# ldyken53/gaussian-splatting-wgpu

Measured on AMD Instinct MI355X. Metric: frames/sec, higher is better.
Workload: dtype f32; 1 GPU; bicycle-like synthetic 6.1M gaussians @1920x1080; gaussians=6100000, width=1920, height=1080, tile_size=16, parallelism=single GPU, visible=2430918, processed=15909895, block_evaluated=6068168, sort_passes=1, depth_ordered_emission=True, tight_binning=True, blend_mode=fused, camera=64-step orbit, moved every frame

## Files before the change

### gaussian-splatting-wgpu_amd/csrc/gs_context.hip

```cpp
#include <cmath>
#include <cstdarg>
#include <memory>
#include <new>

#include "gs_runtime.h"

thread_local char g_err[512] = "";
int32_t fail(int32_t code, const char* fmt, ...) {
    va_list ap;
    va_start(ap, fmt);
    vsnprintf(g_err, sizeof(g_err), fmt, ap);
    va_end(ap);
    return code;
}

static uint32_t tiles_f32(uint32_t extent, uint32_t ts) {
    return (uint32_t)std::ceil((float)extent / (float)ts);
}
static uint32_t bits_for(uint64_t v) {
    uint32_t b = 0;
    while (v) { ++b; v >>= 1; }
    return b ? b : 1;
}

GS_EXPORT const char* gs_last_error(void) { return g_err; }
GS_EXPORT int32_t gs_abi_version(void) { return GS_ABI_VERSION; }

int32_t alloc_kv(gs_ctx* c, uint64_t capacity, uint64_t row_cap) {
    if (capacity >= (1ull << 30)) return fail(GS_ERR_CAPACITY, "capacity %llu exceeds 2^30 intersections", (unsigned long long)capacity);
    if (row_cap >= (1ull << 31)) return fail(GS_ERR_CAPACITY, "%llu row items exceed the 2^31 limit", (unsigned long long)row_cap);
    c->gr.valid = false;
    c->keysA.reset(); c->valsA.reset(); c->keysB.reset(); c->valsB.reset(); c->keysU.reset(); c->valsU.reset();
    c->keysG.reset(); c->chunk_table.reset(); c->arena.reset(); c->rows_sorted.reset(); c->M3.reset(); c->ctl_mem.reset();
    c->keysG_valid = false;
    capacity = std::max<uint64_t>(capacity, 4096);
    row_cap = (std::max<uint64_t>(row_cap, 4096) + 15) & ~(uint64_t)15;
    const size_t kb = (size_t)capacity * 4;
    HIP_TRY(hipMalloc(c->keysA.out(), kb));
    HIP_TRY(hipMalloc(c->valsA.out(), kb));
    HIP_TRY(hipMalloc(c->keysB.out(), kb));
    HIP_TRY(hipMalloc(c->valsB.out(), kb));
    HIP_TRY(hipMalloc(c->chunk_table.out(), (size_t)gs_emit_chunks(std::max(capacity, row_cap)) * 4));
    if (c->tight_ok) {
        HIP_TRY(hipMalloc(c->arena.out(), (size_t)row_cap * 12));
        HIP_TRY(hipMalloc(c->rows_sorted.out(), (size_t)row_cap * 12));
        HIP_TRY(hipMalloc(c->M3.out(), (size_t)gs_rows_chunks(row_cap) * 256 * 4));
    }
    const size_t ctl_sz = (sizeof(GsControl) + 255) & ~(size_t)255;
    const size_t scan_sz = (((size_t)gs_scan_blocks(c->n ? c->n : 1) + 1) * 8 + 255) & ~(size_t)255;
    const size_t sort_sz = (size_t)std::max(c->passes, c->tile_passes) * gs_sort_tiles(capacity) * 256 * 4;
    const size_t rows_sz = c->tight_ok ? (size_t)gs_rows_sort_tiles(row_cap) * 256 * 4 : 0;
    const size_t depth_sz = ((size_t)c->T * 4 + 255) & ~(size_t)255;
    c->ctl_bytes = ctl_sz + depth_sz + rows_sz + scan_sz + sort_sz;
    c->ctl_bytes_tight = ctl_sz + depth_sz + rows_sz;
    HIP_TRY(hipMalloc(c->ctl_mem.out(), c->ctl_bytes));
    char* const base = (char*)c->ctl_mem.get();
    c->ctl = (GsControl*)base;
    c->tile_depth = (uint32_t*)(base + ctl_sz);
    c->rows_status = (uint32_t*)(base + ctl_sz + depth_sz);
    c->scan_status = (unsigned long long*)(base + ctl_sz + depth_sz + rows_sz);
    c->sort_status = (uint32_t*)(base + ctl_sz + depth_sz + rows_sz + scan_sz);
    c->capacity = capacity;
    c->row_cap = row_cap;
    c->frame.capacity = (uint32_t)capacity;
    c->frame.row_cap = (uint32_t)row_cap;
    return GS_OK;
}

GS_EXPORT int32_t gs_create(const gs_config* cfg, gs_ctx** out) {
    if (!cfg || !out) return fail(GS_ERR_INVALID_ARGUMENT, "gs_create: null argument");
    if (cfg->struct_size != sizeof(gs_config)) return fail(GS_ERR_INVALID_ARGUMENT, "gs_create: struct_size %u != %zu", cfg->struct_size, sizeof(gs_config));
    if (cfg->width == 0 || cfg->height == 0) return fail(GS_ERR_INVALID_ARGUMENT, "gs_create: empty canvas");
    if (cfg->tile_size != 8 && cfg->tile_size != 16 && cfg->tile_size != 32)
        return fail(GS_ERR_INVALID_ARGUMENT, "gs_create: tile_size must be 8, 16 or 32 (got %u)", cfg->tile_size);
    int ndev = 0;
    if (hipGetDeviceCount(&ndev) != hipSuccess || ndev == 0) return fail(GS_ERR_NO_DEVICE, "gs_create: no HIP device");
    if (cfg->device < 0 || cfg->device >= ndev) return fail(GS_ERR_INVALID_ARGUMENT, "gs_create: device %d of %d", cfg->device, ndev);
    HIP_TRY(hipSetDevice(cfg->device));

    std::unique_ptr<gs_ctx> c(new (std::nothrow) gs_ctx());
    if (!c) return fail(GS_ERR_OUT_OF_MEMORY, "gs_create: host allocation failed");
    c->cfg = *cfg;
    GsFrame& f = c->frame;
    f.width = cfg->width; f.height = cfg->height; f.tile_size = cfg->tile_size;
    f.ntx = tiles_f32(cfg->width, cfg->tile_size);
    f.nty = tiles_f32(cfg->height, cfg->tile_size);
    if (f.ntx >= 32768 || f.nty >= 65536) return fail(GS_ERR_INVALID_ARGUMENT, "gs_create: canvas too large");
    f.col0 = cfg->col_begin;
    f.col1 = cfg->col_end;
    if (f.col0 == 0 && f.col1 == 0) f.col1 = f.ntx;
    if (f.col1 > f.ntx || f.col0 >= f.col1) return fail(GS_ERR_INVALID_ARGUMENT, "gs_create: bad tile-column slab [%u,%u) of %u", f.col0, f.col1, f.ntx);
    f.full = (f.col0 == 0 && f.col1 == f.ntx) ? 1u : 0u;
    f.px0 = f.col0 * f.tile_size;
    f.slab_w = std::min(f.width, f.col1 * f.tile_size) - f.px0;
    c->T = f.ntx * f.nty;
    const uint64_t max_key = ((uint64_t)f.nty * f.ntx + f.ntx) * 1000ull + 999ull;
    if (max_key > 0xFFFFFFFFull) return fail(GS_ERR_INVALID_ARGUMENT, "gs_create: tile ids overflow the 32-bit key (write_tile_ids.wgsl:29)");
    c->key_bits = bits_for(max_key);
    c->passes = (c->key_bits + 7) / 8;
    const uint32_t tbits = bits_for((uint64_t)f.nty * f.ntx + f.ntx);
    c->tile_passes = (tbits + 7) / 8;
    c->tile_bits = (tbits + c->tile_passes - 1) / c->tile_passes;
    c->tile16 = ((uint64_t)f.nty * f.ntx + f.ntx) < 0xFFFFull;
    if ((uint64_t)(f.ntx + 1) * (f.nty + 1) > GS_COUNT_MASK) return fail(GS_ERR_INVALID_ARGUMENT, "gs_create: canvas has too many tiles");
    c->tight_ok = f.ntx <= 255u && f.nty <= 255u;

    hipDeviceProp_t prop;
    HIP_TRY(hipGetDeviceProperties(&prop, cfg->device));
    c->grid_persist = (uint32_t)prop.multiProcessorCount * 4;
    if (cfg->stream) c->stream = (hipStream_t)cfg->stream;
    else { HIP_TRY(hipStreamCreateWithFlags(c->own_stream.out(), hipStreamNonBlocking)); c->stream = c->own_stream; }

    HIP_TRY(hipMalloc(c->ranges.out(), (size_t)c->T * 4));
    HIP_TRY(hipMemset(c->ranges, 0, (size_t)c->T * 4));
    const size_t px = (size_t)f.slab_w * f.height;
    HIP_TRY(hipMalloc(c->rgba8.out(), px * 4));
    HIP_TRY(hipMemset(c->rgba8, 0, px * 4));
    if (cfg->flags & GS_FLAG_F32_TAP) HIP_TRY(hipMalloc(c->rgbf.out(), px * 12));
    if (cfg->flags & GS_FLAG_AUX_OUTPUTS) {
        HIP_TRY(hipMalloc(c->alpha.out(), px * 4));
        HIP_TRY(hipMalloc(c->depth.out(), px * 4));
        HIP_TRY(hipMemset(c->alpha, 0, px * 4));
        HIP_TRY(hipMemset(c->depth, 0, px * 4));
    }
    HIP_TRY(hipHostMalloc(c->h_ctl.out(), sizeof(GsControl), hipHostMallocDefault));
    memset(c->h_ctl, 0, sizeof(GsControl));
    HIP_TRY(hipMalloc(c->d_pxb.out(), 65 * 4));
    HIP_TRY(hipMalloc(c->tileoff.out(), 256 * 256 * 4));
    HIP_TRY(hipMalloc(c->rowtot.out(), 256 * 4));
    HIP_TRY(hipMalloc(c->sticky.out(), 4 * 4));
    HIP_TRY(hipMemset(c->sticky, 0, 4 * 4));
    HIP_TRY(hipHostMalloc(c->h_rep.out(), sizeof(GsReport), hipHostMallocDefault));
    memset(c->h_rep, 0, sizeof(GsReport));
    if (cfg->flags & GS_FLAG_TIMING) {
        for (auto& row : c->ev)
            for (auto& e : row) HIP_TRY(hipEventCreate(e.out()));
        c->have_events = true;
    }
    c->fif = (c->own_stream && f.full) ? 3u : 1u;
    *out = c.release();
    return GS_OK;
}

gs_ctx::~gs_ctx() { drop_graph(this); }

GS_EXPORT int32_t gs_destroy(gs_ctx* c) {
    if (!c) return GS_OK;
    hipSetDevice(c->cfg.device);
    drop_shadows(c);
    if (c->stream) hipStreamSynchronize(c->stream);
    delete c;
    return GS_OK;
}

static int32_t alloc_per_gaussian(gs_ctx* c, uint64_t n, uint64_t min_capacity = 0, uint64_t min_rows = 0) {
    c->gr.valid = false;
    c->scene_own.reset();
    c->scene_mem = nullptr;
    c->n = (uint32_t)n;
    c->frame.n = (uint32_t)n;
    c->have_frame = false;
    c->counts.reset(); c->offsets.reset(); c->grec.reset(); c->rowptr.reset(); c->gsort_scratch.reset(); c->gdata.reset();
    const size_t np = ((size_t)n + 63) & ~(size_t)63;
    HIP_TRY(hipMalloc(c->counts.out(), std::max<size_t>(np * 4, 256)));
    HIP_TRY(hipMalloc(c->offsets.out(), std::max<size_t>(np * 4, 256)));
    HIP_TRY(hipMalloc(c->grec.out(), std::max<size_t>(np * 16, 256)));
    HIP_TRY(hipMalloc(c->rowptr.out(), std::max<size_t>(np * 4, 256)));
    HIP_TRY(hipMalloc(c->gsort_scratch.out(), gs_gsort_scratch_bytes((uint32_t)n)));
    HIP_TRY(hipMalloc(c->gdata.out(), std::max<size_t>((size_t)n * 64, 256)));
    HIP_TRY(hipMemsetAsync(c->gdata, 0, std::max<size_t>((size_t)n * 64, 256), c->stream));
    uint64_t cap = c->cfg.max_intersections ? c->cfg.max_intersections : std::max<uint64_t>(4 * n, 1u << 22);
    cap = std::max<uint64_t>(cap, min_capacity);
    cap = std::min<uint64_t>(cap, (1ull << 30) - 1);
    const uint64_t rows = std::max<uint64_t>(std::max<uint64_t>(2 * n, 1u << 20), min_rows);
    return alloc_kv(c, cap, rows);
}

int32_t scene_alloc(gs_ctx* c, uint64_t n, uint64_t min_capacity, uint64_t min_rows) {
    int32_t rc = alloc_per_gaussian(c, n, min_capacity, min_rows);
    if (rc != GS_OK) return rc;
    const size_t np = ((size_t)n + 63) & ~(size_t)63;
    const size_t sh_end = np * 4 * 4 + np * 32 + (size_t)n * 192, state_at = (sh_end + 255) & ~(size_t)255;
    const size_t bytes = has_state(c) ? state_at + np : sh_end;
    HIP_TRY(hipMalloc(c->scene_own.out(), std::max<size_t>(bytes, 256)));
    c->scene_mem = c->scene_own;
    c->scene_bytes = bytes;
    char* p = (char*)c->scene_mem;
    GsScene& s = c->scene;
    s.px = (float*)p; p += np * 4; s.py = (float*)p; p += np * 4; s.pz = (float*)p; p += np * 4;
    s.smax = (float*)p; p += np * 4;
    s.geo = (float4*)p; p += np * 32;
    s.sh = (float4*)p;
    s.state = nullptr;
    if (has_state(c)) {
        s.state = (const uint8_t*)c->scene_mem + state_at;
        HIP_TRY(hipMemsetAsync((char*)c->scene_mem + state_at, 0, std::max<size_t>(np, 4), c->stream));
    }
    return GS_OK;
}

static int32_t upload_common(gs_ctx* c, const void* d_aos, uint64_t n) {
    int32_t rc = scene_alloc(c, n);
    if (rc != GS_OK) return rc;
    if (n) gs_launch_repack(d_aos, (uint32_t)n, c->scene, c->stream);
    HIP_TRY(hipGetLastError());
    HIP_TRY(hipStreamSynchronize(c->stream));
    return GS_OK;
}

void drop_shadows(gs_ctx* c) {
    for (gs_ctx* s : c->shadows) gs_destroy(s);
    c->shadows.clear();
    c->last = c;
    c->rr = 0;
    c->cap_hint = 0;
    c->row_hint = 0;
}
GS_EXPORT int32_t gs_share_splats(gs_ctx* c, gs_ctx* owner) {
    if (!c || !owner || c == owner) return fail(GS_ERR_INVALID_ARGUMENT, "gs_share_splats: needs two distinct contexts");
    if (c->cfg.device != owner->cfg.device) return fail(GS_ERR_INVALID_ARGUMENT, "gs_share_splats: contexts are on different devices");
    if (!c->is_shadow) drop_shadows(c);
    if (!owner->scene_mem) return fail(GS_ERR_NO_SCENE, "gs_share_splats: the owner holds no splats");
    if (has_state(c) && !has_state(owner))
        return fail(GS_ERR_INVALID_ARGUMENT, "gs_share_splats: this context has GS_FLAG_SPLAT_STATE, the owner keeps no state plane");
    HIP_TRY(hipSetDevice(c->cfg.device));
    if (c->pending) { int32_t rc = wait_one(c); if (rc != GS_OK) return rc; }
    int32_t rc = alloc_per_gaussian(c, owner->n, c->cfg.max_intersections ? 0 : owner->capacity, owner->row_cap);
    if (rc != GS_OK) return rc;
    c->scene_mem = owner->scene_mem;
    c->scene_bytes = owner->scene_bytes;
    c->scene = owner->scene;
    HIP_TRY(hipStreamSynchronize(c->stream));
    return GS_OK;
}

GS_EXPORT int32_t gs_upload_splats_device(gs_ctx* c, const void* d_aos, uint64_t n) {
    if (!c || (!d_aos && n)) return fail(GS_ERR_INVALID_ARGUMENT, "gs_upload_splats_device: null argument");
    if (n >= (1ull << 31)) return fail(GS_ERR_INVALID_ARGUMENT, "gs_upload_splats: too many gaussians");
    HIP_TRY(hipSetDevice(c->cfg.device));
    drop_shadows(c);
    return upload_common(c, d_aos, n);
}

GS_EXPORT int32_t gs_upload_splats(gs_ctx* c, const void* aos, uint64_t n) {
    if (!c || (!aos && n)) return fail(GS_ERR_INVALID_ARGUMENT, "gs_upload_splats: null argument");
    if (n >= (1ull << 31)) return fail(GS_ERR_INVALID_ARGUMENT, "gs_upload_splats: too many gaussians");
    HIP_TRY(hipSetDevice(c->cfg.device));
    drop_shadows(c);
    DevBuf<> d;
    const size_t bytes = (size_t)n * GS_SPLAT_RECORD_BYTES;
    HIP_TRY(hipMalloc(d.out(), std::max<size_t>(bytes, 256)));
    if (bytes) {
        hipError_t e = hipMemcpy(d, aos, bytes, hipMemcpyHostToDevice);
        if (e != hipSuccess) return fail(GS_ERR_HIP, "upload memcpy: %s", hipGetErrorString(e));
    }
    return upload_common(c, d, n);
}

GS_EXPORT int32_t gs_host_alloc(uint64_t bytes, void** out) {
    if (!out) return fail(GS_ERR_INVALID_ARGUMENT, "gs_host_alloc: null argument");
    *out = nullptr;
    HIP_TRY(hipHostMalloc(out, std::max<size_t>((size_t)bytes, 256), hipHostMallocDefault));
    return GS_OK;
}
GS_EXPORT void gs_host_free(void* p) { if (p) hipHostFree(p); }

GS_EXPORT int32_t gs_slab_width(gs_ctx* c, uint32_t* px_begin, uint32_t* px_width) {
    if (!c) return fail(GS_ERR_INVALID_ARGUMENT, "gs_slab_width: null ctx");
    if (px_begin) *px_begin = c->frame.px0;
    if (px_width) *px_width = c->frame.slab_w;
    return GS_OK;
}

static int32_t set_option_one(gs_ctx* c, int32_t key, int64_t value) {
    c->gr.valid = false;
    switch (key) {
    case GS_OPT_FRAME_GRAPH: c->gr.use = (value != 0); return GS_OK;
    case GS_OPT_BLEND_ABLATION: c->blend_ablation = (uint32_t)value & 0x3FFFFu; return GS_OK;
    case GS_OPT_PERSISTENT_GRID: if (value <= 0) break; c->grid_persist = (uint32_t)value; return GS_OK;
    case GS_OPT_RESET_TIMING: c->timed_from = c->frames; c->max_I_seen = 0; c->truncated_frames = 0; return GS_OK;
    case GS_OPT_EMIT_ORDER: if (value < 0 || value > 2) break; c->emit_order = (int)value; return GS_OK;
    case GS_OPT_UNFUSED: return GS_OK;
    case GS_OPT_DEBUG_VIEW: if (value < 0 || value > 4) break; c->debug_view = (uint32_t)value; return GS_OK;
    case GS_OPT_TILE_CULL: c->tile_cull = (value != 0); return GS_OK;
    case GS_OPT_PROJ_CHUNKS: if (value != 0 && value != 2 && value != 4 && value != 8) break; c->tight_nb = (uint32_t)value; return GS_OK;
    case GS_OPT_SELECT_TINT:
        if (!has_state(c)) return fail(GS_ERR_INVALID_ARGUMENT, "gs_set_option: GS_OPT_SELECT_TINT needs GS_FLAG_SPLAT_STATE");
        if (value < 0 || value > 0xFFFFFFFFll) break;
        c->select_tint = (uint32_t)value;
        return GS_OK;
    default: break;
    }
    return fail(GS_ERR_INVALID_ARGUMENT, "gs_set_option: bad key/value %d/%lld", key, (long long)value);
}
GS_EXPORT int32_t gs_set_option(gs_ctx* c, int32_t key, int64_t value) {
    if (!c) return fail(GS_ERR_INVALID_ARGUMENT, "gs_set_option: null ctx");
    if (key == GS_OPT_FRAMES_IN_FLIGHT) {
        if (value < 1 || value > 4) return fail(GS_ERR_INVALID_ARGUMENT, "gs_set_option: frames in flight must be 1..4");
        if (!c->own_stream || !c->frame.full) value = 1;
        int32_t rc = gs_wait(c);
        if (rc != GS_OK && rc != GS_ERR_TRUNCATED) return rc;
        while (c->shadows.size() + 1 > (size_t)value) {
            if (c->last == c->shadows.back()) { c->last = c; }
            gs_destroy(c->shadows.back());
            c->shadows.pop_back();
        }
        c->fif = (uint32_t)value;
        c->rr = 0;
        return GS_OK;
    }
    int32_t rc = set_option_one(c, key, value);
    for (gs_ctx* s : c->shadows) if (rc == GS_OK) rc = set_option_one(s, key, value);
    return rc;
}
```

### gaussian-splatting-wgpu_amd/csrc/gs_frame.hip

```cpp
#include <dlfcn.h>

#include "gs_runtime.h"
#include "gs_tight.h"

namespace {
struct Roctx {
    int (*push)(const char*) = nullptr;
    int (*pop)() = nullptr;
    Roctx() {
        void* h = dlopen("librocprofiler-sdk-roctx.so.1", RTLD_LAZY | RTLD_LOCAL);
        if (!h) h = dlopen("libroctx64.so.4", RTLD_LAZY | RTLD_LOCAL);
        if (h) {
            push = (int (*)(const char*))dlsym(h, "roctxRangePushA");
            pop = (int (*)())dlsym(h, "roctxRangePop");
            if (!push || !pop) push = nullptr, pop = nullptr;
        }
    }
};
Roctx& roctx() { static Roctx r; return r; }
const char* const kStageRange[] = {"gsplat:process_gaussians", "gsplat:exclusive_scan", "gsplat:write_tile_ids", "gsplat:radix_sort",
                                   "gsplat:compute_ranges", "gsplat:compute_tiles"};
}

static inline void mark(gs_ctx* c, int i) {
    if (!c->have_events) return;
    hipEventRecord(c->ev[c->frames % GS_EV_RING][i], c->stream);
    Roctx& r = roctx();
    if (r.push) {
        if (i > 0) r.pop();
        if (i < GS_STAGE_COUNT) r.push(kStageRange[i]);
    }
}

static void mark_cb(void* p, int i) { mark((gs_ctx*)p, i); }

static int32_t record_frame(gs_ctx* c, const GsUniforms& u, bool debug, void* ext_rgba8, bool tight) {
    const GsFrame& f = c->frame;
    hipStream_t st = c->stream;
    FrameNotes& nt = c->notes;
    gs_launch_zero(c->ctl_mem, tight ? c->ctl_bytes_tight : c->ctl_bytes, st);
    c->h_ctl_valid = false;
    if (debug) HIP_TRY(hipMemsetAsync(c->gdata, 0, std::max<size_t>((size_t)c->n * 64, 256), st));
    mark(c, 0);
    gs_preprocess_prepare(c->pre, c->scene, u, f, c->gdata, c->counts, tight, c->arena, c->rowptr, c->ctl, c->tight_nb, has_state(c),
                          tint_of(c->select_tint));
    gs_launch_preprocess(c->pre, st);
    mark(c, 1);
    const bool by_index = !tight && (debug || c->index_order);
    bool keys16 = false;
    if (tight) {
        gs_launch_gsort(c->counts, c->rowptr, c->n, c->gsort_scratch, c->grec, c->chunk_table, (uint32_t)gs_emit_chunks(std::max(c->capacity, c->row_cap)),
                        &c->ctl->num_visible, &c->ctl->num_slots, c->grid_persist, st);
        mark(c, 2);
        gs_launch_rows(c->arena, c->grec, c->chunk_table, c->rows_sorted, c->ctl, c->rows_status, (uint32_t)c->row_cap, c->M3, c->tileoff, c->rowtot, f, c->valsA,
                       c->ranges, c->grid_persist / 4u, c->sticky, c->h_rep, st, mark_cb, c);
        nt.keysS = nullptr;
        nt.valsS = c->valsA;
        mark(c, 4);
    } else if (by_index) {
        gs_launch_scan(c->counts, c->n, c->offsets, c->scan_status, &c->ctl->scan_ticket[0], c->ctl, st);
        mark(c, 2);
        gs_launch_emit(c->gdata, c->counts, c->offsets, nullptr, nullptr, f, c->keysA, c->valsA, c->ctl, st);
    } else {
        gs_launch_gsort(c->counts, nullptr, c->n, c->gsort_scratch, c->grec, c->chunk_table, (uint32_t)gs_emit_chunks(std::max(c->capacity, c->row_cap)),
                        &c->ctl->num_visible, &c->ctl->num_intersections, c->grid_persist, st);
        mark(c, 2);
        gs_launch_emit_balanced(c->gdata, c->grec, c->chunk_table, f, c->keysA, c->valsA, c->ctl, c->grid_persist * 2,
                                c->tile_bits, c->tile_passes, c->tile16, st);
        keys16 = c->tile16;
    }
    if (debug) {
        if (!c->keysU) {
            HIP_TRY(hipMalloc(c->keysU.out(), (size_t)c->capacity * 4));
            HIP_TRY(hipMalloc(c->valsU.out(), (size_t)c->capacity * 4));
        }
        HIP_TRY(hipMemcpyAsync(c->keysU, c->keysA, (size_t)c->capacity * 4, hipMemcpyDeviceToDevice, st));
        HIP_TRY(hipMemcpyAsync(c->valsU, c->valsA, (size_t)c->capacity * 4, hipMemcpyDeviceToDevice, st));
    }
    if (!tight) {
        mark(c, 3);
        if (by_index)
            gs_launch_sort(c->keysA, c->valsA, c->keysB, c->valsB, c->ctl, c->ctl->sort_ticket, &c->ctl->hist[0][0], &c->ctl->num_intersections,
                           (uint32_t)c->capacity, c->passes, 8, 0, c->sort_status, c->grid_persist, false, nullptr, nullptr, st, &nt.keysS, &nt.valsS);
        else
            gs_launch_sort(c->keysA, c->valsA, c->keysB, c->valsB, c->ctl, c->ctl->sort_ticket, &c->ctl->hist[0][0], &c->ctl->num_intersections,
                           (uint32_t)c->capacity, c->tile_passes, c->tile_bits, keys16 ? 0 : 1, c->sort_status, c->grid_persist, true,
                           nullptr, nullptr, st, &nt.keysS, &nt.valsS, keys16);
        mark(c, 4);
        if (keys16) gs_launch_ranges16((const uint16_t*)nt.keysS, c->ctl, (uint32_t)c->capacity, c->T, c->ranges, c->grid_persist * 2, c->sticky, c->h_rep, st);
        else gs_launch_ranges(nt.keysS, c->ctl, (uint32_t)c->capacity, c->T, c->ranges, c->grid_persist * 2, c->sticky, c->h_rep, st);
    }
    nt.last_passes = tight ? 1u : (by_index ? c->passes : c->tile_passes);
    nt.last_by_index = by_index;
    nt.last_keys16 = keys16;
    nt.last_tight = tight;
    mark(c, 5);
    uint32_t* target = ext_rgba8 ? (uint32_t*)ext_rgba8 : c->rgba8.get();
    if ((c->blend_ablation & 0x10000u) && !c->blend_prof) HIP_TRY(hipMalloc(c->blend_prof.out(), (size_t)(1u << 20) * 16));
    const bool aux = (c->cfg.flags & GS_FLAG_AUX_OUTPUTS) != 0;
    const int walkers = gs_launch_blend(c->gdata, nt.valsS, c->ranges, f, target, c->rgbf, aux, c->alpha, c->depth, c->ctl, c->tile_depth,
                                        (c->cfg.flags & GS_FLAG_EXACT_BLEND) != 0, c->blend_ablation & 0xFFFFu, tight, st,
                                        (c->blend_ablation & 0x10000u) ? c->blend_prof.get() : nullptr, &c->blend_prof_blocks);
    if (walkers == -2) return fail(GS_ERR_INVALID_ARGUMENT, "blend: GS_FLAG_AUX_OUTPUTS without its alpha / depth planes");
    if (walkers < 0) return fail(GS_ERR_INVALID_ARGUMENT, "unsupported tile size %u", f.tile_size);
    nt.blend_walkers = (uint32_t)walkers;
    mark(c, 6);
    if (c->debug_view) gs_launch_debug_view(c->ranges, f, c->debug_view, target, st);
    return GS_OK;
}

void drop_graph(gs_ctx* c) {
    if (c->gr.exec) hipGraphExecDestroy(c->gr.exec);
    if (c->gr.graph) hipGraphDestroy(c->gr.graph);
    c->gr.exec = nullptr; c->gr.graph = nullptr; c->gr.pre_node = nullptr;
    c->gr.valid = false;
}

static int32_t enqueue_frame(gs_ctx* c, const GsUniforms& u, bool debug, void* ext_rgba8) {
    hipStream_t st = c->stream;
    if (c->emit_order == 2) {
        const uint64_t saved = c->passes > c->tile_passes ? c->passes - c->tile_passes : 0;
        c->index_order = !(c->have_frame && saved * (uint64_t)c->h_rep->num_intersections >= 1000000ull);
    } else {
        c->index_order = (c->emit_order == 1);
    }
    const bool tight = !debug && c->tile_cull && c->tight_ok && c->n < (1u << GS_ID_BITS);
    const bool graphable = c->gr.use && !debug && !c->have_events && !(c->blend_ablation & 0x10000u) && c->n;
    if (graphable) {
        const GraphKey key{c->index_order, tight, ext_rgba8, c->alpha, c->depth};
        if (!c->gr.exec || !c->gr.valid || !(c->gr.key == key)) {
            if (c->gr.exec) HIP_TRY(hipStreamSynchronize(st));
            drop_graph(c);
            HIP_TRY(hipStreamBeginCapture(st, hipStreamCaptureModeRelaxed));
            const int32_t rc = record_frame(c, u, debug, ext_rgba8, tight);
            const hipError_t e = hipStreamEndCapture(st, &c->gr.graph);
            if (rc != GS_OK) { drop_graph(c); return rc; }
            if (e != hipSuccess || !c->gr.graph) return fail(GS_ERR_HIP, "frame graph capture: %s", hipGetErrorString(e));
            hipGraph_t g = c->gr.graph;
            HIP_TRY(hipGraphInstantiate(&c->gr.exec, g, nullptr, nullptr, 0));
            size_t nn = 0;
            HIP_TRY(hipGraphGetNodes(g, nullptr, &nn));
            std::vector<hipGraphNode_t> nodes(nn);
            HIP_TRY(hipGraphGetNodes(g, nodes.data(), &nn));
            uint32_t found = 0;
            for (hipGraphNode_t nd : nodes) {
                hipGraphNodeType ty;
                if (hipGraphNodeGetType(nd, &ty) != hipSuccess || ty != hipGraphNodeTypeKernel) continue;
                hipKernelNodeParams kp;
                if (hipGraphKernelNodeGetParams(nd, &kp) == hipSuccess && kp.func == c->pre.func) { c->gr.pre_node = nd; ++found; }
            }
            if (found != 1) {
                c->gr.use = false;
                c->gr.pre_node = nullptr;
            }
            c->gr.key = key;
            c->gr.notes = c->notes;
            c->gr.valid = true;
        } else {
            c->notes = c->gr.notes;
            gs_preprocess_prepare(c->pre, c->scene, u, c->frame, c->gdata, c->counts, tight, c->arena, c->rowptr, c->ctl, c->tight_nb, has_state(c),
                                  tint_of(c->select_tint));
            hipKernelNodeParams kp{};
            kp.func = const_cast<void*>(c->pre.func);
            kp.gridDim = dim3(c->pre.blocks); kp.blockDim = dim3(256); kp.sharedMemBytes = 0;
            kp.kernelParams = c->pre.args; kp.extra = nullptr;
            HIP_TRY(hipGraphExecKernelNodeSetParams(c->gr.exec, c->gr.pre_node, &kp));
        }
        HIP_TRY(hipGraphLaunch(c->gr.exec, st));
        c->gr.frames++;
    } else {
        const int32_t rc = record_frame(c, u, debug, ext_rgba8, tight);
        if (rc != GS_OK) return rc;
    }
    c->keysG_valid = false;
    c->h_ctl_valid = false;
    HIP_TRY(hipGetLastError());
    c->pending = true;
    c->have_frame = true;
    c->last_debug = debug;
    c->last_ext = ext_rgba8;
    c->last_u = u;
    c->frames++;
    return GS_OK;
}

static int32_t render_common(gs_ctx* c, const void* uniforms, bool debug, void* ext) {
    if (!c || !uniforms) return fail(GS_ERR_INVALID_ARGUMENT, "gs_render: null argument");
    if (!c->scene_mem) return fail(GS_ERR_NO_SCENE, "gs_render: no splats uploaded");
    HIP_TRY(hipSetDevice(c->cfg.device));
    GsUniforms u;
    static_assert(sizeof(GsUniforms) == GS_UNIFORM_BYTES, "uniform block must be 160 bytes");
    memcpy(&u, uniforms, sizeof(u));
    return enqueue_frame(c, u, debug, ext);
}

int32_t wait_one(gs_ctx* c) {
    if (!c) return fail(GS_ERR_INVALID_ARGUMENT, "gs_wait: null ctx");
    HIP_TRY(hipSetDevice(c->cfg.device));
    uint32_t dropped = 0;
    for (int attempt = 0; attempt < 8; ++attempt) {
        HIP_TRY(hipStreamSynchronize(c->stream));
        c->pending = false;
        if (!c->have_frame) return GS_OK;
        const uint32_t over_frames = c->h_rep->sticky[0], fault_any = c->h_rep->sticky[1];
        const uint64_t max_I = c->h_rep->sticky[2], max_rows = c->h_rep->sticky[3];
        if (over_frames || fault_any || max_I || max_rows) HIP_TRY(hipMemset(c->sticky, 0, 4 * 4));
        c->h_rep->sticky[0] = c->h_rep->sticky[1] = c->h_rep->sticky[2] = c->h_rep->sticky[3] = 0;
        if (max_I > c->max_I_seen) c->max_I_seen = max_I;
        if (fault_any || c->h_rep->fault) return fail(GS_ERR_DEVICE_FAULT, "a look-back spin exceeded its bound (fault word set)");
        const uint64_t I = c->h_rep->num_intersections;
        uint64_t rows_last = 0;
        if (c->notes.last_tight)
            for (int k = 0; k < 16; ++k) rows_last = std::max<uint64_t>(rows_last, (uint64_t)c->h_rep->row_cursor[k] * 16);
        const bool last_over = I > c->capacity || c->h_rep->overflow;
        if (attempt == 0 && over_frames > (last_over ? 1u : 0u)) dropped = over_frames - (last_over ? 1u : 0u);
        const uint64_t need = std::max<uint64_t>(I, max_I), need_rows = std::max<uint64_t>(rows_last, max_rows);
        if (!last_over && need <= c->capacity && need_rows <= c->row_cap) break;
        if (need >= (1ull << 30)) return fail(GS_ERR_CAPACITY, "%llu intersections exceed the 2^30 limit", (unsigned long long)need);
        uint64_t want = c->capacity, want_rows = c->row_cap;
        if (need > c->capacity) want = std::min<uint64_t>(std::max<uint64_t>(need + need / 4, c->capacity * 2), (1ull << 30) - 1);
        if (need_rows > c->row_cap) want_rows = std::max<uint64_t>(need_rows + need_rows / 4, c->row_cap * 2);
        if (want == c->capacity && want_rows == c->row_cap) {
            if (last_over) return fail(GS_ERR_CAPACITY, "the frame reports an overflow that growing cannot fix (capacity %llu, rows %llu)",
                                       (unsigned long long)c->capacity, (unsigned long long)c->row_cap);
            break;
        }
        int32_t rc = alloc_kv(c, want, want_rows);
        if (rc != GS_OK) return rc;
        if (!last_over) break;
        if (attempt == 7) return fail(GS_ERR_CAPACITY, "capacity did not converge");
        c->frames--;
        rc = enqueue_frame(c, c->last_u, c->last_debug, c->last_ext);
        if (rc != GS_OK) return rc;
    }
    if (dropped) {
        c->truncated_frames += dropped;
        return fail(GS_ERR_TRUNCATED, "%u frame(s) enqueued before the last one overflowed the (key,value) capacity and were rendered from "
                    "truncated lists; the capacity has been grown to %llu -- wait after every frame, or pass gs_config.max_intersections",
                    dropped, (unsigned long long)c->capacity);
    }
    return GS_OK;
}

GS_EXPORT int32_t gs_wait(gs_ctx* c) {
    if (!c) return fail(GS_ERR_INVALID_ARGUMENT, "gs_wait: null ctx");
    int32_t first = wait_one(c);
    char msg[sizeof(g_err)];
    if (first != GS_OK) memcpy(msg, g_err, sizeof(msg));
    for (gs_ctx* s : c->shadows) {
        const int32_t rc = wait_one(s);
        if (rc != GS_OK && first == GS_OK) { first = rc; memcpy(msg, g_err, sizeof(msg)); }
    }
    c->cap_hint = std::max(c->cap_hint, c->capacity);
    c->row_hint = std::max(c->row_hint, c->row_cap);
    for (gs_ctx* s : c->shadows) { c->cap_hint = std::max(c->cap_hint, s->capacity); c->row_hint = std::max(c->row_hint, s->row_cap); }
    if (first != GS_OK) memcpy(g_err, msg, sizeof(msg));
    return first;
}

static int32_t add_shadow(gs_ctx* c) {
    gs_config cfg = c->cfg;
    cfg.stream = nullptr;
    cfg.max_intersections = 0;
    gs_ctx* s = nullptr;
    int32_t rc = gs_create(&cfg, &s);
    if (rc != GS_OK) return rc;
    s->fif = 1;
    s->is_shadow = true;
    rc = gs_share_splats(s, c);
    if (rc != GS_OK) { gs_destroy(s); return rc; }
    s->emit_order = c->emit_order; s->tile_cull = c->tile_cull; s->debug_view = c->debug_view;
    s->blend_ablation = c->blend_ablation; s->grid_persist = c->grid_persist; s->timed_from = 0; s->tight_nb = c->tight_nb;
    s->select_tint = c->select_tint;
    s->gr.use = c->gr.use;
    c->shadows.push_back(s);
    return GS_OK;
}

GS_EXPORT int32_t gs_render(gs_ctx* c, const void* uniforms) {
    if (!c || !uniforms) return fail(GS_ERR_INVALID_ARGUMENT, "gs_render: null argument");
    gs_ctx* t = c;
    if (c->fif > 1 && c->scene_mem) {
        if (c->pending && c->shadows.size() + 1 < c->fif) {
            int32_t rc = add_shadow(c);
            if (rc != GS_OK) return rc;
            c->rr = (uint32_t)c->shadows.size();
        }
        if (!c->shadows.empty()) {
            const uint32_t slot = c->rr++ % (uint32_t)(c->shadows.size() + 1);
            t = slot ? c->shadows[slot - 1] : c;
        }
        if (t->capacity < c->cap_hint || t->row_cap < c->row_hint) {
            HIP_TRY(hipSetDevice(t->cfg.device));
            if (t->pending) { int32_t rc = wait_one(t); if (rc != GS_OK && rc != GS_ERR_TRUNCATED) return rc; }
            int32_t rc = alloc_kv(t, std::max(t->capacity, c->cap_hint), std::max(t->row_cap, c->row_hint));
            if (rc != GS_OK) return rc;
            t->have_frame = false;
        }
    }
    const int32_t rc = render_common(t, uniforms, false, nullptr);
    if (rc == GS_OK) c->last = t;
    return rc;
}
GS_EXPORT int32_t gs_render_debug(gs_ctx* c, const void* uniforms) {
    const int32_t rc = render_common(c, uniforms, true, nullptr);
    if (rc == GS_OK && c) c->last = c;
    return rc;
}
GS_EXPORT int32_t gs_render_to(gs_ctx* c, const void* uniforms, void* d_rgba8) {
    if (!d_rgba8) return fail(GS_ERR_INVALID_ARGUMENT, "gs_render_to: null output");
    const int32_t rc = render_common(c, uniforms, false, d_rgba8);
    if (rc == GS_OK && c) c->last = c;
    return rc;
}

GS_EXPORT int32_t gs_render_host(gs_ctx* c, const void* uniforms, void* host_dst, uint64_t size, uint64_t* ticket) {
    if (!c || !uniforms || !host_dst || !ticket) return fail(GS_ERR_INVALID_ARGUMENT, "gs_render_host: null argument");
    const uint64_t bytes = (uint64_t)c->frame.slab_w * c->frame.height * 4;
    if (size < bytes) return fail(GS_ERR_INVALID_ARGUMENT, "gs_render_host: need %llu bytes, got %llu", (unsigned long long)bytes, (unsigned long long)size);
    int32_t rc = gs_render(c, uniforms);
    if (rc != GS_OK) return rc;
    gs_ctx* t = last_of(c);
    if (!t->ev_done) HIP_TRY(hipEventCreateWithFlags(t->ev_done.out(), hipEventDisableTiming));
    HIP_TRY(hipMemcpyAsync(host_dst, t->rgba8, bytes, hipMemcpyDeviceToHost, t->stream));
    std::lock_guard<std::mutex> lk(c->ticket_mu);
    HIP_TRY(hipEventRecord(t->ev_done, t->stream));
    const uint64_t k = c->next_ticket++;
    c->tickets[k & 63u].ticket = k;
    c->tickets[k & 63u].member = t;
    *ticket = k;
    return GS_OK;
}

GS_EXPORT int32_t gs_wait_ticket(gs_ctx* c, uint64_t ticket) {
    if (!c) return fail(GS_ERR_INVALID_ARGUMENT, "gs_wait_ticket: null ctx");
    gs_ctx* t = nullptr;
    {
        std::lock_guard<std::mutex> lk(c->ticket_mu);
        if (ticket == 0 || ticket >= c->next_ticket) return fail(GS_ERR_INVALID_ARGUMENT, "gs_wait_ticket: unknown ticket %llu", (unsigned long long)ticket);
        if (c->next_ticket - ticket > 64 || c->tickets[ticket & 63u].ticket != ticket) return GS_OK;
        t = c->tickets[ticket & 63u].member;
    }
    HIP_TRY(hipSetDevice(c->cfg.device));
    HIP_TRY(hipEventSynchronize(t->ev_done));
    return GS_OK;
}
```

### gaussian-splatting-wgpu_amd/csrc/gs_kernels.h

```cpp
#pragma once
#include "gs_device.h"

void gs_launch_repack(const void* d_aos, uint32_t n, const GsScene& s, hipStream_t st);
void gs_launch_ply_chunk(const void* d_raw, uint32_t m, uint32_t first, const GsPlyTable& t, const GsScene& s, hipStream_t st);
struct GsPreprocessLaunch {
    const void* func;
    uint32_t blocks;
    GsScene s; GsUniforms u; GsFrame f;
    void* gdata; uint32_t* counts; GsTightOut to; GsTint tint;
    void* args[7];
};
void gs_preprocess_prepare(GsPreprocessLaunch& L, const GsScene& s, const GsUniforms& u, const GsFrame& f, void* gdata, uint32_t* counts,
                           bool tight, uint32_t* arena, uint32_t* rowptr, GsControl* ctl, uint32_t tight_nb = 0, bool state = false,
                           GsTint tint = GsTint{});
void gs_launch_preprocess(GsPreprocessLaunch& L, hipStream_t st);
void gs_launch_zero(void* p, uint64_t bytes, hipStream_t st);
uint32_t gs_scan_blocks(uint32_t n);
void gs_launch_scan(const uint32_t* counts, uint32_t n, uint32_t* offsets, unsigned long long* status, uint32_t* ticket, GsControl* ctl,
                    hipStream_t st);
uint64_t gs_emit_chunks(uint64_t capacity);
void gs_launch_emit_balanced(const void* gdata, const void* grec, const uint32_t* chunk_table, const GsFrame& f, uint32_t* keys, uint32_t* values,
                             GsControl* ctl, uint32_t grid, uint32_t hist_bits, uint32_t hist_passes, bool keys16, hipStream_t st);
void gs_launch_emit(const void* gdata, const uint32_t* counts, const uint32_t* offsets, const uint32_t* perm, const uint32_t* n_dev,
                    const GsFrame& f, uint32_t* keys, uint32_t* values, GsControl* ctl, hipStream_t st);
void gs_launch_ranges16(const uint16_t* tiles, const GsControl* ctl, uint32_t capacity, uint32_t T, uint32_t* ranges, uint32_t grid,
                        uint32_t* sticky, GsReport* rep, hipStream_t st);
void gs_launch_rebuild_keys(const uint16_t* tiles, const uint32_t* vals, const uint32_t* counts, uint32_t count, uint32_t n, uint32_t id_mask,
                            uint32_t* keys, hipStream_t st);
void gs_launch_ranges(const uint32_t* keys, const GsControl* ctl, uint32_t capacity, uint32_t T, uint32_t* ranges, uint32_t grid,
                      uint32_t* sticky, GsReport* rep, hipStream_t st);
uint32_t gs_sort_tiles(uint64_t capacity);
void gs_launch_sort(uint32_t* keysA, uint32_t* valsA, uint32_t* keysB, uint32_t* valsB, GsControl* ctl, uint32_t* tickets, uint32_t* hist,
                    const uint32_t* n_ptr, uint32_t capacity, uint32_t passes, uint32_t bits, uint32_t by_tile, uint32_t* status,
                    uint32_t grid, bool have_hist, const uint32_t* aux_table, uint32_t* aux_out, hipStream_t st, uint32_t** out_keys,
                    uint32_t** out_vals, bool keys16 = false);
int gs_launch_blend(const void* gdata, const uint32_t* values, const uint32_t* ranges, const GsFrame& f, uint32_t* rgba8, float* rgbf,
                    bool aux, float* alpha, float* depth, GsControl* ctl, uint32_t* tile_depth, bool exact, uint32_t ablation, bool masked, hipStream_t st, uint32_t* prof = nullptr,
                    uint32_t* prof_blocks = nullptr);
void gs_launch_debug_view(const uint32_t* ranges, const GsFrame& f, uint32_t view, uint32_t* rgba8, hipStream_t st);
void gs_launch_assemble(const void* slabs, void* image, uint32_t width, uint32_t height, const uint32_t* d_px_bounds, uint32_t n_slabs,
                        uint64_t slab_stride_px, hipStream_t st);
uint32_t gs_gsort_tiles(uint32_t n);
uint64_t gs_gsort_scratch_bytes(uint32_t n);
void gs_launch_gsort(const uint32_t* words, const uint32_t* aux_in, uint32_t n, void* scratch, void* grec, uint32_t* chunk_table, uint32_t chunk_cap,
                     uint32_t* tot_visible, uint32_t* tot_quantity, uint32_t grid, hipStream_t st);
uint32_t gs_rows_sort_tiles(uint64_t row_cap);
uint32_t gs_rows_chunks(uint64_t row_cap);
void gs_launch_rows(const uint32_t* arena, const void* grec, const uint32_t* chunk_table, uint32_t* rows_sorted, GsControl* ctl, uint32_t* sort_status, uint32_t row_cap,
                    uint32_t* M3, uint32_t* tileoff, uint32_t* rowtot, const GsFrame& f, uint32_t* values, uint32_t* ranges, uint32_t cus,
                    uint32_t* sticky, GsReport* rep, hipStream_t st, void (*mark)(void*, int), void* mark_arg);
void gs_launch_rows_rebuild_keys(const uint32_t* ranges, uint32_t T, const uint32_t* vals, const uint32_t* counts, uint32_t count, uint32_t n,
                                 uint32_t* keys, hipStream_t st);
struct GsRegionDev {
    float a[3], b[3];
    float x0, y0, x1, y1;
    float W, H;
    uint32_t wi, hi;
    float proj[16];
    float viewz[4];
    const uint8_t* mask;
};
#define GS_STATE_SLOTS 32
#define GS_STATE_SLOT_STRIDE 32
void gs_launch_state_region(uint32_t kind, uint8_t* state, const GsScene& s, uint32_t n, const GsRegionDev& r, uint32_t op, uint32_t bits,
                            uint32_t where_mask, uint32_t where_value, unsigned long long* matched, hipStream_t st);
void gs_launch_state_ids(uint8_t* state, const uint32_t* ids, uint64_t n, uint32_t op, uint32_t bits, hipStream_t st);
void gs_launch_state_count(const uint8_t* state, uint32_t n, uint32_t mask, uint32_t value, unsigned long long* count, hipStream_t st);
uint32_t gs_select_blocks(uint32_t n);
void gs_launch_select_count(const uint8_t* state, uint32_t n, uint32_t mask, uint32_t value, uint32_t* counts, hipStream_t st);
void gs_launch_select_scatter(const uint8_t* state, uint32_t n, uint32_t mask, uint32_t value, const uint32_t* offsets, uint32_t* ids, uint32_t cap,
                              hipStream_t st);
void gs_launch_unpack(const GsScene& s, uint32_t n, const uint32_t* ids, uint32_t first, uint32_t m, void* d_aos, uint32_t* out_ids, hipStream_t st);
void gs_launch_compact_planes(const GsScene& o, uint32_t n_old, const uint32_t* ids, uint32_t m, const GsScene& d, hipStream_t st);
void gs_launch_pick(const void* gdata, const uint32_t* values, const uint32_t* ranges, const GsFrame& f, uint32_t id_mask, const void* d_queries,
                    uint32_t n, void* d_results, uint32_t max_contrib, void* d_contrib, hipStream_t st);
```

### gaussian-splatting-wgpu_amd/csrc/gs_runtime.h

```cpp
#pragma once
#include <hip/hip_runtime.h>

#include <algorithm>
#include <cstdint>
#include <cstdio>
#include <cstring>
#include <mutex>
#include <vector>

#include "../../include/gsplat/gs_abi.h"
#include "gs_kernels.h"

#define GS_EXPORT extern "C" __attribute__((visibility("default")))

extern thread_local char g_err[512];
int32_t fail(int32_t code, const char* fmt, ...) __attribute__((format(printf, 2, 3)));
#define HIP_TRY(expr)                                                                                       \
    do {                                                                                                    \
        hipError_t e_ = (expr);                                                                             \
        if (e_ != hipSuccess)                                                                               \
            return fail(e_ == hipErrorOutOfMemory ? GS_ERR_OUT_OF_MEMORY : GS_ERR_HIP, "%s: %s", #expr,      \
                        hipGetErrorString(e_));                                                             \
    } while (0)

template <class P, auto Destroy>
struct Owned {
    P p = nullptr;
    Owned() = default;
    explicit Owned(P q) : p(q) {}
    Owned(const Owned&) = delete;
    Owned& operator=(const Owned&) = delete;
    Owned(Owned&& o) noexcept : p(o.p) { o.p = nullptr; }
    Owned& operator=(Owned&& o) noexcept { if (this != &o) { reset(); p = o.p; o.p = nullptr; } return *this; }
    ~Owned() { reset(); }
    void reset() { if (p) { (void)Destroy(p); p = nullptr; } }
    P* out() { reset(); return &p; }
    P get() const { return p; }
    operator P() const { return p; }
    P operator->() const { return p; }
};
template <class T = void> using DevBuf = Owned<T*, hipFree>;
template <class T = void> using PinnedBuf = Owned<T*, hipHostFree>;
using Event = Owned<hipEvent_t, hipEventDestroy>;
using Stream = Owned<hipStream_t, hipStreamDestroy>;
using File = Owned<FILE*, fclose>;

struct FrameNotes {
    uint32_t *keysS = nullptr, *valsS = nullptr;
    uint32_t last_passes = 0;
    uint32_t blend_walkers = 1;
    bool last_by_index = true;
    bool last_keys16 = false;
    bool last_tight = false;
};

struct GraphKey {
    bool index = false, tight = false;
    void* ext = nullptr;
    float *alpha = nullptr, *depth = nullptr;
    bool operator==(const GraphKey& o) const { return index == o.index && tight == o.tight && ext == o.ext && alpha == o.alpha && depth == o.depth; }
};

#define GS_EV_RING 256
struct gs_ctx {
    ~gs_ctx();
    gs_config cfg{};
    Stream own_stream;
    hipStream_t stream = nullptr;
    GsFrame frame{};
    uint32_t T = 0, passes = 0, key_bits = 0;
    uint32_t tile_passes = 0, tile_bits = 0;
    bool tile16 = false;
    bool tight_ok = false;
    uint32_t grid_persist = 0;
    int emit_order = 2;
    bool index_order = true;
    uint32_t debug_view = 0;
    bool tile_cull = true;
    uint32_t tight_nb = 0;
    uint32_t blend_ablation = 0;
    uint32_t select_tint = 0x80FFFF00u;
    DevBuf<uint32_t> blend_prof;
    uint32_t blend_prof_blocks = 0;
    uint32_t fif = 1;
    std::vector<gs_ctx*> shadows;
    bool is_shadow = false;
    gs_ctx* last = nullptr;
    uint32_t rr = 0;
    uint64_t cap_hint = 0, row_hint = 0;
    Event ev_done;
    uint64_t next_ticket = 1;
    struct { uint64_t ticket; gs_ctx* member; } tickets[64] = {};
    std::mutex ticket_mu;
    DevBuf<> scene_own;
    void* scene_mem = nullptr;
    size_t scene_bytes = 0;
    GsScene scene{};
    uint32_t n = 0;
    DevBuf<uint32_t> counts, offsets, rowptr;
    DevBuf<> gdata;
    DevBuf<> grec;
    DevBuf<> gsort_scratch;
    uint64_t capacity = 0;
    DevBuf<uint32_t> keysA, valsA, keysB, valsB;
    DevBuf<uint32_t> keysU, valsU;
    DevBuf<uint32_t> keysG;
    bool keysG_valid = false;
    DevBuf<uint32_t> chunk_table;
    uint64_t row_cap = 0;
    DevBuf<uint32_t> arena, rows_sorted, M3;
    DevBuf<uint32_t> tileoff, rowtot;
    DevBuf<> ctl_mem;
    size_t ctl_bytes = 0;
    size_t ctl_bytes_tight = 0;
    GsControl* ctl = nullptr;
    uint32_t* tile_depth = nullptr;
    uint32_t* rows_status = nullptr;
    unsigned long long* scan_status = nullptr;
    uint32_t* sort_status = nullptr;
    PinnedBuf<GsControl> h_ctl;
    bool h_ctl_valid = false;
    PinnedBuf<GsReport> h_rep;
    DevBuf<uint32_t> sticky;
    uint64_t max_I_seen = 0;
    uint64_t truncated_frames = 0;
    DevBuf<uint32_t> ranges, rgba8;
    DevBuf<float> rgbf;
    DevBuf<float> alpha, depth;
    DevBuf<uint32_t> d_pxb;
    uint32_t pxb_host[65] = {};
    uint32_t pxb_n = 0;
    struct { DevBuf<> q, r, c; uint64_t c_bytes = 0; } pick;
    struct { DevBuf<unsigned long long> counter; DevBuf<uint32_t> ids; DevBuf<uint8_t> mask; uint64_t ids_cap = 0, mask_cap = 0; } st;
    struct { DevBuf<uint32_t> counts, ids; uint64_t counts_cap = 0, ids_cap = 0; } ex;
    Event ev[GS_EV_RING][GS_STAGE_COUNT + 1];
    bool have_events = false;
    uint64_t timed_from = 0;
    struct {
        bool use = false, valid = false;
        hipGraph_t graph = nullptr;
        hipGraphExec_t exec = nullptr;
        hipGraphNode_t pre_node = nullptr;
        GraphKey key;
        FrameNotes notes;
        uint64_t frames = 0;
    } gr;
    GsPreprocessLaunch pre{};
    FrameNotes notes;
    bool have_frame = false, pending = false, last_debug = false;
    void* last_ext = nullptr;
    GsUniforms last_u{};
    uint64_t frames = 0;
};

int32_t alloc_kv(gs_ctx* c, uint64_t capacity, uint64_t row_cap);
int32_t scene_alloc(gs_ctx* c, uint64_t n, uint64_t min_capacity = 0, uint64_t min_rows = 0);
void drop_shadows(gs_ctx* c);
void drop_graph(gs_ctx* c);
int32_t wait_one(gs_ctx* c);
inline gs_ctx* last_of(gs_ctx* c) { return (c && c->last) ? c->last : c; }
inline bool has_state(const gs_ctx* c) { return (c->cfg.flags & GS_FLAG_SPLAT_STATE) != 0; }
inline GsTint tint_of(uint32_t argb) {
    return GsTint{{(float)((argb >> 16) & 255u) / 255.0f, (float)((argb >> 8) & 255u) / 255.0f, (float)(argb & 255u) / 255.0f},
                  (float)(argb >> 24) / 255.0f};
}
```

### gaussian-splatting-wgpu_amd/csrc/gs_tight.h

```cpp
#pragma once
#include "gs_device.h"

#define GS_ID_BITS 28
#define GS_ID_MASK 0x0FFFFFFFu

struct TightG {
    float gx, gy;
    float cx, cy, cz;
    float cxz;
    float lim2;
    float rcx;
    float xmax, ymax;
    float dyR, eR;
    float kc, qa, qb;
    uint32_t mode;
};

__device__ __forceinline__ bool tight_finite(float x) { return __builtin_fabsf(x) < 3.0e38f; }

__device__ __forceinline__ TightG tight_setup(float uvx, float uvy, float cx, float cy, float cz, float op, float Wf, float Hf) {
    TightG g;
    g.gx = uvx * Wf;
    g.gy = uvy * Hf;
    g.cx = cx; g.cy = cy; g.cz = cz;
    g.cxz = cx * cz;
    const float cyy = cy * cy;
    const float D = g.cxz - cyy;
    const float errD = 4.0e-7f * (g.cxz + cyy);
    const float lim = __builtin_amdgcn_logf(op * 255.0f) * 0.693147182464599609375f + 0.01f;
    g.lim2 = 2.0f * lim;
    g.rcx = 1.0f / cx;
    g.xmax = 0.0f; g.ymax = 0.0f; g.dyR = 0.0f; g.eR = 0.0f;
    g.kc = -(cy * g.rcx);
    g.qa = (cyy - g.cxz) + 1.0e-5f * (cyy + g.cxz);
    g.qb = (g.lim2 * cx) * 1.00001f;
    const bool pd = (cx > 0.0f) && (cz > 0.0f) && (D > 0.0f);
    const bool fin = tight_finite(g.gx) && tight_finite(g.gy) && tight_finite(cx) && tight_finite(cy) && tight_finite(cz) && tight_finite(g.rcx);
    if (!fin) { g.mode = 2u; return g; }
    if (lim < 0.0f) { g.mode = 0u; return g; }
    const float Dlo = D - 1.1e-5f * (g.cxz + cyy) - errD;
    if (!pd || !fin || !tight_finite(lim) || !(Dlo > 0.25f * D)) { g.mode = 2u; return g; }
    g.xmax = __builtin_sqrtf(g.lim2 * 1.0001f * cz / Dlo) * 1.0002f + 0.02f;
    g.ymax = __builtin_sqrtf(g.lim2 * 1.0001f * cx / Dlo) * 1.0002f + 0.02f;
    g.dyR = -cy * g.xmax / cz;
    g.eR = __builtin_fabsf(g.dyR) * ((D - Dlo) / Dlo + 4.0e-4f) + 0.02f;
    g.mode = tight_finite(g.xmax) && tight_finite(g.ymax) && tight_finite(g.dyR) ? 1u : 2u;
    return g;
}

__device__ __forceinline__ bool tight_chord(const TightG& g, float dy, float& xlo, float& xhi) {
    const float up = __builtin_fmaf(dy * dy, g.qa, g.qb);
    if (!(up >= 0.0f)) return false;
    const float hw = __builtin_amdgcn_sqrtf(up) * g.rcx;
    const float c = g.kc * dy;
    xlo = c - hw;
    xhi = c + hw;
    return true;
}

__device__ __forceinline__ bool tight_strip(const TightG& g, float a, float b, bool va, float lo_a, float hi_a, bool vb, float lo_b,
                                            float hi_b, float& plo, float& phi) {
    float xlo, xhi;
    if (!va && !vb) {
        if (!(a <= 0.0f && 0.0f <= b)) return false;
        xlo = -g.xmax;
        xhi = g.xmax;
    } else {
        xlo = va ? (vb ? __builtin_fminf(lo_a, lo_b) : lo_a) : lo_b;
        xhi = va ? (vb ? __builtin_fmaxf(hi_a, hi_b) : hi_a) : hi_b;
        if (g.dyR >= a - g.eR && g.dyR <= b + g.eR) xhi = g.xmax;
        if (-g.dyR >= a - g.eR && -g.dyR <= b + g.eR) xlo = -g.xmax;
    }
    const float slack = 0.02f + 1.0e-5f * (__builtin_fabsf(xlo) + __builtin_fabsf(xhi) + __builtin_fabsf(g.gx));
    plo = g.gx - xhi - slack;
    phi = g.gx - xlo + slack;
    return true;
}

__device__ __forceinline__ void tight_cols(float plo, float phi, float w, float inv_w, int cmin, int cmax, int& lo, int& hi) {
    const float flo = __builtin_ceilf((plo - (w - 1.0f)) * inv_w), fhi = __builtin_floorf(phi * inv_w);
    lo = flo <= (float)cmin ? cmin : (flo > (float)cmax ? cmax + 1 : (int)flo);
    hi = fhi >= (float)cmax ? cmax : (fhi < (float)cmin ? cmin - 1 : (int)fhi);
}

struct TightChord { bool v; float lo, hi; };
__device__ __forceinline__ TightChord tight_chord_at(const TightG& g, float dy) {
    TightChord c;
    c.lo = c.hi = 0.0f;
    c.v = tight_chord(g, dy, c.lo, c.hi);
    return c;
}
__device__ __forceinline__ float tight_row_dy(const TightG& g, uint32_t ty, uint32_t ts) { return g.gy - (float)(ty * ts); }

__device__ __forceinline__ void tight_rows(const TightG& g, uint32_t y0, uint32_t y1, uint32_t ts, float inv_ts, uint32_t nty, uint32_t alias,
                                           uint32_t& ra, uint32_t& rb) {
    if (y1 > nty) y1 = nty;
    ra = y0; rb = y1 > y0 ? y1 : y0;
    if (g.mode != 1u) return;
    const float lo = __builtin_floorf((g.gy - g.ymax) * inv_ts) - (alias ? 1.0f : 0.0f), hi = __builtin_floorf((g.gy + g.ymax) * inv_ts) + 1.0f;
    if (lo > (float)ra) ra = lo >= (float)rb ? rb : (uint32_t)lo;
    if (hi < (float)rb) rb = hi <= (float)ra ? ra : (uint32_t)hi;
}

struct TightRow { int tlo, thi; uint32_t alias; };
__device__ __forceinline__ uint32_t tight_row(const TightG& g, uint32_t ty, uint32_t ts, float inv_ts, uint32_t nty, uint32_t xa, uint32_t wmain,
                                              uint32_t alias, const TightChord& cb, const TightChord& ca, TightRow& r) {
    r.tlo = 0; r.thi = -1; r.alias = 0u;
    if (ty >= nty) return 0u;
    if (wmain) {
        if (g.mode == 2u) { r.tlo = (int)xa; r.thi = (int)(xa + wmain) - 1; }
        else {
            float plo, phi;
            if (tight_strip(g, tight_row_dy(g, ty + 1u, ts), tight_row_dy(g, ty, ts), ca.v, ca.lo, ca.hi, cb.v, cb.lo, cb.hi, plo, phi))
                tight_cols(plo, phi, (float)ts, inv_ts, (int)xa, (int)(xa + wmain) - 1, r.tlo, r.thi);
            else { r.tlo = (int)xa; r.thi = (int)xa - 1; }
        }
    }
    if (alias && ty + 1u < nty) {
        if (g.mode == 2u) r.alias = 1u;
        else {
            const TightChord c2 = tight_chord_at(g, tight_row_dy(g, ty + 2u, ts));
            float plo, phi;
            int lo = 1, hi = 0;
            if (tight_strip(g, tight_row_dy(g, ty + 2u, ts), tight_row_dy(g, ty + 1u, ts), c2.v, c2.lo, c2.hi, ca.v, ca.lo, ca.hi, plo, phi))
                tight_cols(plo, phi, (float)ts, inv_ts, 0, 0, lo, hi);
            r.alias = lo <= hi ? 1u : 0u;
        }
    }
    return (uint32_t)(r.thi >= r.tlo ? r.thi - r.tlo + 1 : 0) + r.alias;
}

__device__ __forceinline__ uint32_t tight_count(const TightG& g, uint32_t y0, uint32_t y1, uint32_t ts, float inv_ts, uint32_t nty, uint32_t xa,
                                                uint32_t wmain, uint32_t alias) {
    if (g.mode == 0u) return 0u;
    uint32_t ra, rb, n = 0;
    tight_rows(g, y0, y1, ts, inv_ts, nty, alias, ra, rb);
    if (ra >= rb) return 0u;
    TightRow r;
    TightChord cb = tight_chord_at(g, tight_row_dy(g, ra, ts));
    for (uint32_t ty = ra; ty < rb; ++ty) {
        const TightChord ca = tight_chord_at(g, tight_row_dy(g, ty + 1u, ts));
        n += tight_row(g, ty, ts, inv_ts, nty, xa, wmain, alias, cb, ca, r);
        cb = ca;
    }
    return n;
}

__device__ __forceinline__ void tight_substrips(const TightG& g, uint32_t ty, uint32_t ts, uint32_t sub, float inv_sub, int cmin, int cmax,
                                                const TightChord& cb, const TightChord& ca, int lo[2], int hi[2]) {
    lo[0] = lo[1] = cmax + 1; hi[0] = hi[1] = cmin - 1;
    if (g.mode == 2u) { lo[0] = lo[1] = cmin; hi[0] = hi[1] = cmax; return; }
    const float yb = tight_row_dy(g, ty, ts), ya = tight_row_dy(g, ty + 1u, ts);
    float plo, phi;
    if (sub == ts) {
        if (tight_strip(g, ya, yb, ca.v, ca.lo, ca.hi, cb.v, cb.lo, cb.hi, plo, phi)) tight_cols(plo, phi, (float)sub, inv_sub, cmin, cmax, lo[0], hi[0]);
        return;
    }
    const float ym = g.gy - (float)(ty * ts + sub);
    const TightChord cm = tight_chord_at(g, ym);
    if (tight_strip(g, ym, yb, cm.v, cm.lo, cm.hi, cb.v, cb.lo, cb.hi, plo, phi)) tight_cols(plo, phi, (float)sub, inv_sub, cmin, cmax, lo[0], hi[0]);
    if (tight_strip(g, ya, ym, ca.v, ca.lo, ca.hi, cm.v, cm.lo, cm.hi, plo, phi)) tight_cols(plo, phi, (float)sub, inv_sub, cmin, cmax, lo[1], hi[1]);
}

#define GS_ROW_HOLE 0xFFFFFFFFu
#define GS_ROW_MAX_DIM 255u
__device__ __forceinline__ uint32_t tight_enc8(int v) { return v <= 0 ? 0u : (v >= 255 ? 255u : (uint32_t)v); }
__device__ __forceinline__ uint32_t tight_pack_intervals(const int lo[2], const int hi[2], int cmin, uint32_t ncols) {
    if (ncols > 254u) return 0xFF00FF00u;
    uint32_t w = 0;
#pragma unroll
    for (int s = 0; s < 2; ++s) {
        uint32_t l = 0, h = 0;
        if (lo[s] <= hi[s]) { l = tight_enc8(lo[s] - cmin); h = tight_enc8(hi[s] + 1 - cmin); }
        w |= (l | (h << 8)) << (16 * s);
    }
    return w;
}
__device__ __forceinline__ uint32_t tight_slot_item(const TightG& g, uint32_t slot, uint32_t ra, uint32_t nrows, uint32_t ts, float inv_ts, uint32_t sub,
                                                    float inv_sub, uint32_t ns, uint32_t nty, uint32_t xa, uint32_t wmain, uint32_t alias, uint32_t& w1,
                                                    uint32_t& w2) {
    w1 = 0u; w2 = 0u;
    TightRow r;
    int lo[2], hi[2];
    if (slot < nrows) {
        const uint32_t ty = ra + slot;
        if (ty >= nty || !wmain) return 0u;
        const int cmin = (int)(xa * ns), cmax = (int)((xa + wmain) * ns) - 1;
        const TightChord cb = tight_chord_at(g, tight_row_dy(g, ty, ts)), ca = tight_chord_at(g, tight_row_dy(g, ty + 1u, ts));
        tight_substrips(g, ty, ts, sub, inv_sub, cmin, cmax, cb, ca, lo, hi);
        int slo = cmax + 1, shi = cmin - 1;
#pragma unroll
        for (int h = 0; h < 2; ++h)
            if (lo[h] <= hi[h]) { slo = lo[h] < slo ? lo[h] : slo; shi = hi[h] > shi ? hi[h] : shi; }
        if (slo > shi) return 0u;
        const uint32_t tlo = (uint32_t)slo / ns, thi = (uint32_t)shi / ns, len = thi - tlo + 1u;
        w1 = ty | (tlo << 8) | ((len - 1u) << 16);
        w2 = tight_pack_intervals(lo, hi, (int)(tlo * ns), len * ns);
        return len;
    }
    if (!alias) return 0u;
    const uint32_t ty = ra + (slot - nrows);
    const TightChord cb = tight_chord_at(g, tight_row_dy(g, ty, ts)), ca = tight_chord_at(g, tight_row_dy(g, ty + 1u, ts));
    if (!tight_row(g, ty, ts, inv_ts, nty, xa, 0u, 1u, cb, ca, r)) return 0u;
    const TightChord c2 = tight_chord_at(g, tight_row_dy(g, ty + 2u, ts));
    tight_substrips(g, ty + 1u, ts, sub, inv_sub, 0, (int)ns - 1, ca, c2, lo, hi);
    w1 = (ty + 1u);
    w2 = tight_pack_intervals(lo, hi, 0, ns);
    return 1u;
}
__device__ __forceinline__ uint32_t tight_item_mask(uint32_t w2, uint32_t q, uint32_t ns) {
    const uint32_t l0 = w2 & 0xFFu, h0 = (w2 >> 8) & 0xFFu, l1 = (w2 >> 16) & 0xFFu, h1 = w2 >> 24;
    if (ns == 2u) {
        const uint32_t c0 = 2u * q, c1 = c0 + 1u;
        return (uint32_t)(l0 <= c0 && (c0 < h0 || h0 == 255u)) | ((uint32_t)(l0 <= c1 && (c1 < h0 || h0 == 255u)) << 1) |
               ((uint32_t)(l1 <= c0 && (c0 < h1 || h1 == 255u)) << 2) | ((uint32_t)(l1 <= c1 && (c1 < h1 || h1 == 255u)) << 3);
    }
    return (uint32_t)(l0 <= q && (q < h0 || h0 == 255u));
}
```

### gaussian-splatting-wgpu_amd/csrc/k_blend.hip

```cpp
#include "gs_device.h"
#include "gs_tight.h"
#include <type_traits>

__device__ __forceinline__ float block_qmin(float cx, float cy, float cz, float dxlo, float dxhi, float dylo, float dyhi,
                                            float& mag) {
    const float X = __builtin_fminf(__builtin_fmaxf(0.0f, dxlo), dxhi);
    const float Y = __builtin_fminf(__builtin_fmaxf(0.0f, dylo), dyhi);
    float q = 3.0e38f;
    mag = 0.0f;
    if (X == 0.0f && Y == 0.0f) return 0.0f;
    if (X != 0.0f) {
        const float dy = __builtin_fminf(__builtin_fmaxf(-cy * X * __builtin_amdgcn_rcpf(cz), dylo), dyhi);
        const float a = 0.5f * cx * X * X, b = 0.5f * cz * dy * dy, c = cy * X * dy;
        q = a + b + c;
        mag = __builtin_fabsf(a) + __builtin_fabsf(b) + __builtin_fabsf(c);
    }
    if (Y != 0.0f) {
        const float dx = __builtin_fminf(__builtin_fmaxf(-cy * Y * __builtin_amdgcn_rcpf(cx), dxlo), dxhi);
        const float a = 0.5f * cx * dx * dx, b = 0.5f * cz * Y * Y, c = cy * dx * Y;
        const float q2 = a + b + c;
        if (q2 < q) { q = q2; mag = __builtin_fabsf(a) + __builtin_fabsf(b) + __builtin_fabsf(c); }
    }
    return q;
}

__device__ __forceinline__ bool blend_tmax_cull(float cx, float cy, float cz, float op, float dxlo, float dxhi, float dylo, float dyhi, float Tmax) {
    const float ax0 = (0.5f * cx) * dxlo * dxlo, ax1 = (0.5f * cx) * dxhi * dxhi, by0 = (0.5f * cz) * dylo * dylo, by1 = (0.5f * cz) * dyhi * dyhi;
    const float c00 = cy * dxlo * dylo, c01 = cy * dxlo * dyhi, c10 = cy * dxhi * dylo, c11 = cy * dxhi * dyhi;
    const float qmax = __builtin_fmaxf(__builtin_fmaxf(ax0 + by0 + c00, ax0 + by1 + c01), __builtin_fmaxf(ax1 + by0 + c10, ax1 + by1 + c11));
    const float qmag = __builtin_fmaxf(ax0, ax1) + __builtin_fmaxf(by0, by1) +
                       __builtin_fmaxf(__builtin_fmaxf(__builtin_fabsf(c00), __builtin_fabsf(c01)), __builtin_fmaxf(__builtin_fabsf(c10), __builtin_fabsf(c11)));
    const float alo = 0.99f * __builtin_fminf(0.99f, op * __builtin_amdgcn_exp2f(-1.44269502162933349609375f * (qmax + 1.0e-5f * qmag)));
    return Tmax * (1.0f - alo) < 0.0000999f;
}

struct GsAuxPlanes { float* alpha; float* depth; };
__device__ __forceinline__ GsAuxPlanes gs_aux_planes() { return GsAuxPlanes{nullptr, nullptr}; }
__device__ __forceinline__ GsAuxPlanes gs_aux_planes(GsAuxPlanes p) { return p; }

template <int TS, bool EXACT, bool AUX = false, typename... Aux>
__global__ __launch_bounds__(TS* TS) void gs_blend_kernel(const uint4* __restrict__ gdata, const uint32_t* __restrict__ values,
                                                           const uint32_t* __restrict__ ranges, GsFrame f,
                                                           uint32_t* __restrict__ rgba8, float* __restrict__ rgbf, GsControl* ctl,
                                                           uint32_t dbg, uint32_t id_mask, Aux... aux) {
    static_assert(sizeof...(Aux) == (AUX ? 1u : 0u), "AUX kernels take one GsAuxPlanes, the others none");
    constexpr int NT = TS * TS;
    constexpr int ROUNDS = NT / 64;
    constexpr int WPR = TS / 8;
    __shared__ float4 sP0[2][NT];
    __shared__ float4 sP1[2][NT];
    __shared__ float4 sP2[2][NT];

    const uint32_t tid = threadIdx.x, lane = tid & 63, w = tid >> 6;
    const uint32_t tx = f.col0 + blockIdx.x, ty = blockIdx.y;
    const uint32_t tile = tx + ty * f.ntx;
    const uint32_t start = tile > 0 ? ranges[tile - 1] : 0u;
    uint32_t end = ranges[tile];
    if (end > f.capacity) end = f.capacity;

    const uint32_t bx0 = tx * TS + (w % WPR) * 8, by0 = ty * TS + (w / WPR) * 8;
    const uint32_t gx = bx0 + (lane & 7), gy = by0 + (lane >> 3);
    const float pxf = (float)gx, pyf = (float)gy;
    const float bx0f = (float)bx0, by0f = (float)by0;
    float T = 1.0f, cr = 0.0f, cg = 0.0f, cb = 0.0f;
    float cd = 0.0f;
    const bool outside = !(gx < f.width && gy < f.height);
    bool done = outside;
    const float c255 = (float)(1.0 / 255.0);
    const float Wf = (float)f.width, Hf = (float)f.height;
    uint32_t staged = 0, evaluated = 0;

    const uint32_t piece = lane & 3u, qrec = lane >> 2;
    uint4 rq[4];
    uint32_t gnext = 0;
    auto fetch_ids = [&](uint32_t b) { gnext = (b + tid < end) ? values[b + tid] : 0u; };
    auto fetch = [&](uint32_t b, uint32_t gval) {
#pragma unroll
        for (int i = 0; i < 4; ++i) {
            const uint32_t rec = qrec + 16u * i;
            uint32_t g = __shfl(gval, rec, 64) & id_mask;
#ifdef GS_PROFILING
            if (dbg & 2u) g &= 1023u;
#endif
            if (b + w * 64u + rec < end && piece < 3u) rq[i] = gdata[(uint64_t)g * 4 + piece];
        }
    };
    auto stage = [&](uint32_t b, int buf) {
#pragma unroll
        for (int i = 0; i < 4; ++i) {
            const uint32_t e = w * 64u + qrec + 16u * i;
            if (b + e < end) {
                const float x = __uint_as_float(rq[i].x), y = __uint_as_float(rq[i].y), z = __uint_as_float(rq[i].z),
                            ww = __uint_as_float(rq[i].w);
                if (piece == 0u) {
                    sP0[buf][e].x = x * Wf;
                    sP0[buf][e].y = y * Hf;
                } else if (piece == 1u) {
                    const float L = 1.44269502162933349609375f;
                    sP1[buf][e] = EXACT ? make_float4(x, y, z, ww) : make_float4((-0.5f * L) * x, (-L) * y, (-0.5f * L) * z, ww);
                } else if (piece == 2u) {
                    sP2[buf][e] = make_float4(x, y, z, ww);
                    sP0[buf][e].z = __builtin_amdgcn_logf(ww * 255.0f) * 0.693147182464599609375f + 0.01f;
                }
            }
        }
    };

    uint32_t gcur = 0;
    if (start < end) {
        fetch_ids(start);
        gcur = gnext;
        fetch(start, gcur);
        fetch_ids(start + NT);
        stage(start, 0);
    }
    __syncthreads();
    int buf = 0;
    for (uint32_t b = start; b < end; b += NT, buf ^= 1) {
        const uint32_t nb = b + NT;
        if (nb < end) {
            gcur = gnext;
            fetch(nb, gcur);
            fetch_ids(nb + NT);
        }
        const uint32_t cnt = (end - b < (uint32_t)NT) ? end - b : (uint32_t)NT;
        staged += cnt;
        const unsigned long long lv = __ballot(!done);
        if (lv != 0ull) {
            uint32_t lcm = (uint32_t)lv | (uint32_t)(lv >> 32);
            lcm |= lcm >> 16; lcm |= lcm >> 8; lcm &= 0xFFu;
            const float lc0 = (float)__builtin_ctz(lcm | 0x100u), lc1 = (float)(31 - __builtin_clz(lcm | 1u));
            const float lr0 = (float)(__builtin_ctzll(lv) >> 3), lr1 = (float)((63 - __builtin_clzll(lv)) >> 3);
            const float Tmax = __uint_as_float((uint32_t)__builtin_amdgcn_readlane((int)wave_incl_max(done ? 0u : __float_as_uint(T)), 63));
#pragma unroll 1
            for (int r = 0; r < ROUNDS; ++r) {
                const uint32_t e0 = (uint32_t)r * 64u;
                if (e0 >= cnt) break;
                bool rel = false;
                if (e0 + lane < cnt) {
                    const float4 p0 = sP0[buf][e0 + lane];
                    float4 p1 = sP1[buf][e0 + lane];
                    if (!EXACT) {
                        const float iL = 0.693147182464599609375f;
                        p1.x *= -2.0f * iL;
                        p1.y *= -iL;
                        p1.z *= -2.0f * iL;
                    }
                    const float dxh = p0.x - bx0f, dyh = p0.y - by0f;
                    const float dxlo = dxh - lc1, dxhi = dxh - lc0, dylo = dyh - lr1, dyhi = dyh - lr0;
                    const bool pd = (p1.x > 0.0f) && (p1.z > 0.0f) && (p1.x * p1.z - p1.y * p1.y > 0.0f);
                    float mag;
                    const float q = block_qmin(p1.x, p1.y, p1.z, dxlo, dxhi, dylo, dyhi, mag);
                    const bool nocull = (dbg & 4u) != 0u;
                    rel = nocull || !pd || !(q > p0.z + 1.0e-5f * mag);
                    if (rel && pd && !nocull && blend_tmax_cull(p1.x, p1.y, p1.z, sP2[buf][e0 + lane].w, dxlo, dxhi, dylo, dyhi, Tmax)) rel = false;
#ifdef GS_PROFILING
                    if (dbg & 1u) rel = false;
#endif
                }
                unsigned long long m = __ballot(rel);
                evaluated += (uint32_t)__popcll(m);
                while (m) {
                    const uint32_t e = e0 + (uint32_t)__builtin_ctzll(m);
                    m &= m - 1ull;
                    const float4 p0 = sP0[buf][e];
                    const float4 p1 = sP1[buf][e];
                    const float4 p2v = sP2[buf][e];
                    const float dx = p0.x - pxf, dy = p0.y - pyf;
                    if (EXACT) {
                        const float t1 = p1.x * dx * dx, t2 = p1.z * dy * dy, t3 = p1.y * dx * dy;
                        const float power = -0.5f * (t1 + t2) - t3;
                        const float alpha = wg_min(0.99f, p2v.w * gs_exp(power));
                        const float test = T * (1.0f - alpha);
                        const float cond = (power <= 0.0f && alpha >= c255 && test >= 0.0001f) ? 1.0f : 0.0f;
                        cr += cond * p2v.x * alpha * T;
                        cg += cond * p2v.y * alpha * T;
                        cb += cond * p2v.z * alpha * T;
                        if constexpr (AUX) cd += cond * p1.w * alpha * T;
                        T = cond * test + (1.0f - cond) * T;
                    } else {
                        const float u = __builtin_fmaf(p1.x, dx, p1.y * dy);
                        const float v = (p1.z * dy) * dy;
                        const float pw = __builtin_fmaf(dx, u, v);
                        const float alpha = __builtin_fminf(0.99f, p2v.w * __builtin_amdgcn_exp2f(pw));
                        const float test = __builtin_fmaf(-T, alpha, T);
                        const bool keep = (pw <= 0.0f) && (alpha >= c255) && (test >= 0.0001f);
                        const float ak = keep ? alpha : 0.0f;
                        const float wgt = ak * T;
                        cr = __builtin_fmaf(p2v.x, wgt, cr);
                        cg = __builtin_fmaf(p2v.y, wgt, cg);
                        cb = __builtin_fmaf(p2v.z, wgt, cb);
                        if constexpr (AUX) cd = __builtin_fmaf(p1.w, wgt, cd);
                        T = keep ? test : T;
                    }
                }
            }
            if (EXACT) done = outside || (T * (1.0f - c255) < 0.0001f);
            else done = outside || (__builtin_fmaf(-T, c255, T) < 0.0001f);
        }
        if (nb < end) stage(nb, buf ^ 1);
        if (__syncthreads_and(done ? 1 : 0)) break;
    }
    if (tid == 0 && staged) atomicAdd(&ctl->num_processed[(blockIdx.x + blockIdx.y * gridDim.x) & 63u], (unsigned long long)staged);
    if (lane == 0 && evaluated) atomicAdd(&ctl->num_evaluated[(blockIdx.x + blockIdx.y * gridDim.x + w) & 63u], (unsigned long long)evaluated);

    if (!outside) {
        const float c[3] = {cr, cg, cb};
        uint32_t q = 0xFF000000u;
#pragma unroll
        for (int ch = 0; ch < 3; ++ch) {
            float v = c[ch];
            v = (v != v) ? 0.0f : wg_min(wg_max(v, 0.0f), 1.0f);
            q |= (uint32_t)__builtin_floorf(v * 255.0f + 0.5f) << (8 * ch);
        }
        const uint64_t o = (uint64_t)gy * f.slab_w + (gx - f.px0);
        rgba8[o] = q;
        if (rgbf) {
            rgbf[o * 3 + 0] = cr;
            rgbf[o * 3 + 1] = cg;
            rgbf[o * 3 + 2] = cb;
        }
        if constexpr (AUX) {
            const GsAuxPlanes ap = gs_aux_planes(aux...);
            ap.alpha[o] = 1.0f - T;
            ap.depth[o] = cd;
        }
    }
}

#ifdef GS_PROFILING
__device__ unsigned long long gs_blend_foot[256][16];
extern "C" __attribute__((visibility("default"))) int gs_prof_blend_footprint(unsigned long long* out4, int reset) {
    static unsigned long long h[256][16];
    if (out4) {
        if (hipMemcpyFromSymbol(h, HIP_SYMBOL(gs_blend_foot), sizeof(h)) != hipSuccess) return -1;
        for (int k = 0; k < 11; ++k) { out4[k] = 0; for (int c = 0; c < 256; ++c) out4[k] += h[c][k]; }
    }
    if (reset) { for (auto& r : h) for (auto& v : r) v = 0; if (hipMemcpyToSymbol(HIP_SYMBOL(gs_blend_foot), h, sizeof(h)) != hipSuccess) return -1; }
    return 0;
}
#endif
constexpr bool gs_lds_disjoint(int a, int na, int b, int nb) { return a + na <= b || b + nb <= a; }
typedef uint32_t gs_u32x2 __attribute__((ext_vector_type(2)));
typedef uint32_t gs_u32x3 __attribute__((ext_vector_type(3)));
typedef uint32_t gs_u32x4 __attribute__((ext_vector_type(4)));
template <bool EXACT, int TS = 16, bool MASKED = false, bool AUX = false, typename... Aux>
__global__ __launch_bounds__(64) void gs_blend_quad_kernel(const uint4* __restrict__ gdata, const uint32_t* __restrict__ values,
                                                            const uint32_t* __restrict__ ranges, GsFrame f,
                                                            uint32_t* __restrict__ rgba8, float* __restrict__ rgbf, GsControl* ctl,
                                                            uint32_t* __restrict__ tile_depth, uint32_t dbg, uint32_t* __restrict__ prof,
                                                            Aux... aux) {
    static_assert(sizeof...(Aux) == (AUX ? 1u : 0u), "AUX kernels take one GsAuxPlanes, the others none");
    constexpr uint32_t BPR = TS / 8, NB = BPR * BPR;
#ifdef GS_PROFILING
    const uint32_t t_start = prof ? (uint32_t)__builtin_amdgcn_s_memrealtime() : 0u;
#endif
#ifndef GS_L_OFF_T
#define GS_L_OFF_T 0
#define GS_L_OFF_Q 4160
#define GS_L_OFF_P 5184
#define GS_L_OFF_L 6208
#define GS_L_TOTAL 6464
#endif
#define GS_L_OFF_Z GS_L_TOTAL
#define GS_L_TOTAL_AUX (GS_L_TOTAL + 256)
    static_assert(gs_lds_disjoint(GS_L_OFF_T, 8 * 65 * 8, GS_L_OFF_Q, 256 * 4) && gs_lds_disjoint(GS_L_OFF_T, 8 * 65 * 8, GS_L_OFF_P, 64 * 16) &&
                  gs_lds_disjoint(GS_L_OFF_T, 8 * 65 * 8, GS_L_OFF_L, 64 * 4) && gs_lds_disjoint(GS_L_OFF_T, 8 * 65 * 8, GS_L_OFF_Z, 64 * 4) &&
                  gs_lds_disjoint(GS_L_OFF_Q, 256 * 4, GS_L_OFF_P, 64 * 16) && gs_lds_disjoint(GS_L_OFF_Q, 256 * 4, GS_L_OFF_L, 64 * 4) &&
                  gs_lds_disjoint(GS_L_OFF_Q, 256 * 4, GS_L_OFF_Z, 64 * 4) && gs_lds_disjoint(GS_L_OFF_P, 64 * 16, GS_L_OFF_L, 64 * 4) &&
                  gs_lds_disjoint(GS_L_OFF_P, 64 * 16, GS_L_OFF_Z, 64 * 4) && gs_lds_disjoint(GS_L_OFF_L, 64 * 4, GS_L_OFF_Z, 64 * 4),
                  "fused LDS regions overlap");
    static_assert(GS_L_OFF_T + 8 * 65 * 8 <= GS_L_TOTAL && GS_L_OFF_Q + 256 * 4 <= GS_L_TOTAL && GS_L_OFF_P + 64 * 16 <= GS_L_TOTAL &&
                  GS_L_OFF_L + 64 * 4 <= GS_L_TOTAL && GS_L_OFF_Z + 64 * 4 <= GS_L_TOTAL_AUX && GS_L_OFF_P % 16 == 0 && GS_L_OFF_T % 8 == 0,
                  "a fused LDS region ends outside its array");
    __shared__ __attribute__((aligned(16))) unsigned char lds_x[EXACT ? 4096 : 16];
    __shared__ __attribute__((aligned(16))) unsigned char lds_f[EXACT ? 16 : (AUX ? GS_L_TOTAL_AUX : GS_L_TOTAL)];
    float4* const sP0 = reinterpret_cast<float4*>(EXACT ? lds_x : lds_f + GS_L_OFF_P);
    float4* const sP1 = reinterpret_cast<float4*>(lds_x + (EXACT ? 1024 : 0));
    float4* const sP2 = reinterpret_cast<float4*>(lds_x + (EXACT ? 2048 : 0));
    uint32_t* const sQ = reinterpret_cast<uint32_t*>(EXACT ? lds_x + 3072 : lds_f + GS_L_OFF_Q);
    float* const sL = reinterpret_cast<float*>(lds_f + (EXACT ? 0 : GS_L_OFF_L));
    float2* const sT = reinterpret_cast<float2*>(lds_f + (EXACT ? 0 : GS_L_OFF_T));
    float* const sZ = reinterpret_cast<float*>(lds_f + ((EXACT || !AUX) ? 0 : GS_L_OFF_Z));
    const uint32_t lane = threadIdx.x;
    const uint32_t slab_tx = f.col1 - f.col0;
    const uint32_t b = blockIdx.x;
    const uint32_t x = b & 7u, j = b >> 3, q = j % NB, t = j / NB;
    const uint32_t SW = (dbg >> 8) & 0xffu;
    const uint32_t ns = (slab_tx + SW - 1) / SW;
    if (x >= ns) return;
    const uint32_t n_x = (ns - 1 - x) / 8 + 1;
    const uint32_t lastw = slab_tx - (ns - 1) * SW;
    const uint32_t Wx = n_x * SW - ((((ns - 1) & 7u) == x) ? SW - lastw : 0u);
    if (t >= Wx * f.nty) return;
    const uint32_t ty = t / Wx, cc = t % Wx;
    const uint32_t tx = f.col0 + (x + 8u * (cc / SW)) * SW + cc % SW;
    const uint32_t lin = ty * slab_tx + (tx - f.col0);
    const uint32_t tile = tx + ty * f.ntx;
    const uint32_t start = tile > 0 ? ranges[tile - 1] : 0u;
    uint32_t end = ranges[tile];
    if (end > f.capacity) end = f.capacity;
    const float c255 = (float)(1.0 / 255.0);
    const float Wf = (float)f.width, Hf = (float)f.height;
    const uint32_t bx0 = tx * TS + (q % BPR) * 8u, by0 = ty * TS + (q / BPR) * 8u;
    const uint32_t gx = bx0 + (lane & 7), gy = by0 + (lane >> 3);
    const float pxf = (float)gx, pyf = (float)gy, bx0f = (float)bx0, by0f = (float)by0;
    const bool outside = !(gx < f.width && gy < f.height);
    bool done = outside;
    float T = 1.0f, cr = 0.0f, cg = 0.0f, cb = 0.0f;
    float cd = 0.0f;
    uint32_t staged = 0, evaluated = 0;
#ifdef GS_PROFILING
    uint32_t fp_lanes = 0, fp_quads = 0, fp_none = 0, fp_live = 0, fp_kept = 0, fp_dead = 0, fp_q1 = 0, fp_tailn = 0, fp_tailbits = 0, fp_nokeep = 0;
#endif

    using R1 = std::conditional_t<AUX, gs_u32x4, gs_u32x3>;
    gs_u32x2 r0 = {0u, 0u};
    R1 r1 = {0u, 0u, 0u};
    gs_u32x4 r2 = {0u, 0u, 0u, 0u};
    const uint32_t mybit = GS_ID_BITS + (TS == 32 ? ((q / BPR) / 2u) * 2u + ((q % BPR) / 2u) : q);
    uint32_t qhead = 0, qn = 0;
    uint32_t pos = start;
    uint32_t g0 = 0, g1 = 0, g2 = 0;
    const __amdgpu_buffer_rsrc_t list_rsrc = __builtin_amdgcn_make_buffer_rsrc((void*)(values + start), 0, (int)((end - start) * 4u), 0x00020000);
    const uint32_t lane4 = lane * 4u;
    auto load_ids = [&]() {
        const uint32_t so = (pos - start) * 4u;
        g0 = __builtin_amdgcn_raw_buffer_load_b32(list_rsrc, lane4, so, 0);
        g1 = __builtin_amdgcn_raw_buffer_load_b32(list_rsrc, lane4 + 256u, so, 0);
        g2 = __builtin_amdgcn_raw_buffer_load_b32(list_rsrc, lane4 + 512u, so, 0);
    };
    const uint32_t mybitmask = 1u << mybit;
    auto push = [&](uint32_t v, uint32_t first) {
        bool want;
        if (MASKED) want = (v & mybitmask) != 0u;
        else want = first + lane < end;
        const unsigned long long m = __ballot(want);
        if (want) sQ[__builtin_amdgcn_mbcnt_hi((uint32_t)(m >> 32), __builtin_amdgcn_mbcnt_lo((uint32_t)m, qhead + qn)) & 255u] = v;
        qn += (uint32_t)__popcll(m);
    };
    auto fill = [&]() {
        while (qn < 64u && pos < end) {
            push(g0, pos); push(g1, pos + 64u); push(g2, pos + 128u);
            const uint32_t adv = end - pos < 192u ? end - pos : 192u;
            staged += adv;
            pos += adv;
            if (pos < end) load_ids();
        }
        __builtin_amdgcn_fence(__ATOMIC_RELEASE, "wavefront");
        __builtin_amdgcn_fence(__ATOMIC_ACQUIRE, "wavefront");
    };
    auto take = [&](uint32_t& v) -> uint32_t {
        const uint32_t cnt = qn < 64u ? qn : 64u;
        v = sQ[(qhead + lane) & 255u];
        qhead = (qhead + cnt) & 255u;
        qn -= cnt;
        return cnt;
    };
    auto fetch = [&](uint32_t v, uint32_t cnt) {
        uint32_t g = MASKED ? (v & GS_ID_MASK) : v;
#ifdef GS_PROFILING
        if (dbg & 2u) g &= 1023u;
#endif
        g = lane < cnt ? g : 0u;
        const uint32_t* rec = reinterpret_cast<const uint32_t*>(gdata + (uint64_t)g * 4);
        r0 = *reinterpret_cast<const gs_u32x2*>(rec);
        r1 = *reinterpret_cast<const R1*>(rec + 4);
        r2 = *reinterpret_cast<const gs_u32x4*>(rec + 8);
    };
    uint32_t cnt = 0, vnext = 0;
    if (start < end) {
        load_ids();
        fill();
        cnt = take(vnext);
        fetch(vnext, cnt);
    }
    while (cnt) {
        bool rel = false, npd = false;
        asm volatile("" : "+v"(r0), "+v"(r1), "+v"(r2));
        const float gxp = __uint_as_float(r0.x) * Wf, gyp = __uint_as_float(r0.y) * Hf;
        const float cx = __uint_as_float(r1.x), cy = __uint_as_float(r1.y), cz = __uint_as_float(r1.z);
        const float op = __uint_as_float(r2.w);
        float z = 0.0f;
        if constexpr (AUX) z = __uint_as_float(r1.w);
        const unsigned long long lv = __ballot(!done);
        uint32_t lcm = (uint32_t)lv | (uint32_t)(lv >> 32);
        lcm |= lcm >> 16; lcm |= lcm >> 8; lcm &= 0xFFu;
        const float lc0 = (float)__builtin_ctz(lcm | 0x100u), lc1 = (float)(31 - __builtin_clz(lcm | 1u));
        const float lr0 = (float)(__builtin_ctzll(lv | (1ull << 63)) >> 3), lr1 = (float)((63 - __builtin_clzll(lv | 1ull)) >> 3);
        const float Tmax = __uint_as_float((uint32_t)__builtin_amdgcn_readlane((int)wave_incl_max(done ? 0u : __float_as_uint(T)), 63));
        if (lane < cnt) {
            const float lim = __builtin_amdgcn_logf(op * 255.0f) * 0.693147182464599609375f + 0.01f;
            const bool pd = (cx > 0.0f) && (cz > 0.0f) && (cx * cz - cy * cy > 0.0f);
            {
                const float dxh = gxp - bx0f, dyh = gyp - by0f;
                float mag;
                const float qm = block_qmin(cx, cy, cz, dxh - lc1, dxh - lc0, dyh - lr1, dyh - lr0, mag);
                const bool nocull = (dbg & 4u) != 0u;
                rel = lv != 0ull && (nocull || !pd || !(qm > lim + 1.0e-5f * mag));
#ifndef GS_NO_TMAX
                if (rel && pd && !nocull) {
                    const float x0 = dxh - lc1, x1 = dxh - lc0, y0 = dyh - lr1, y1 = dyh - lr0;
                    const float ax0 = (0.5f * cx) * x0 * x0, ax1 = (0.5f * cx) * x1 * x1, by0 = (0.5f * cz) * y0 * y0, by1 = (0.5f * cz) * y1 * y1;
                    const float c00 = cy * x0 * y0, c01 = cy * x0 * y1, c10 = cy * x1 * y0, c11 = cy * x1 * y1;
                    const float qmax = __builtin_fmaxf(__builtin_fmaxf(ax0 + by0 + c00, ax0 + by1 + c01), __builtin_fmaxf(ax1 + by0 + c10, ax1 + by1 + c11));
                    const float qmag = __builtin_fmaxf(ax0, ax1) + __builtin_fmaxf(by0, by1) +
                                       __builtin_fmaxf(__builtin_fmaxf(__builtin_fabsf(c00), __builtin_fabsf(c01)), __builtin_fmaxf(__builtin_fabsf(c10), __builtin_fabsf(c11)));
                    const float alo = 0.99f * __builtin_fminf(0.99f, op * __builtin_amdgcn_exp2f(-1.44269502162933349609375f * (qmax + 1.0e-5f * qmag)));
                    if (Tmax * (1.0f - alo) < 0.0000999f) rel = false;
                }
#endif
#ifdef GS_BLEND_PIXTEST
                if (rel && pd && !nocull && (uint32_t)__popcll(lv) <= GS_BLEND_PIXTEST) {
                    bool any = false;
                    for (unsigned long long mm = lv; mm; mm &= mm - 1ull) {
                        const int pl = __builtin_ctzll(mm);
                        const float Tp = __uint_as_float((uint32_t)__builtin_amdgcn_readlane((int)__float_as_uint(T), pl));
                        const float dx = dxh - (float)(pl & 7), dy = dyh - (float)(pl >> 3);
                        const float a = (0.5f * cx) * dx * dx, b = (0.5f * cz) * dy * dy, c = cy * dx * dy;
                        const float q = a + b + c, mg = 1.0e-5f * (a + b + __builtin_fabsf(c));
                        const float ahi = 1.01f * (op * __builtin_amdgcn_exp2f(-1.44269502162933349609375f * (q - mg)));
                        const float alo = 0.99f * __builtin_fminf(0.99f, op * __builtin_amdgcn_exp2f(-1.44269502162933349609375f * (q + mg)));
                        any = any || !(ahi < c255 || Tp * (1.0f - alo) < 0.0000999f);
                    }
                    rel = any;
                }
#endif
            }
#ifdef GS_PROFILING
            if (dbg & 1u) rel = false;
#endif
            npd = rel && !pd;
        }
#ifdef GS_PROFILING
        if ((dbg & 32u) && MASKED && __popcll(lv) <= 16) {
            const unsigned long long rm = __ballot(rel);
            const uint32_t bits = __popc((vnext >> GS_ID_BITS) & 15u);
            fp_tailn += (uint32_t)__popcll(rm);
            fp_tailbits += (uint32_t)__popcll(__ballot(rel && bits >= 1u)) + (uint32_t)__popcll(__ballot(rel && bits >= 2u)) + (uint32_t)__popcll(__ballot(rel && bits >= 3u)) + (uint32_t)__popcll(__ballot(rel && bits >= 4u));
        }
#endif
        const unsigned long long m = __ballot(rel);
        if (rel) {
            const uint32_t slot = __builtin_amdgcn_mbcnt_hi((uint32_t)(m >> 32), __builtin_amdgcn_mbcnt_lo((uint32_t)m, 0u));
            const float L = 1.44269502162933349609375f;
            if (EXACT) {
                sP0[slot] = make_float4(gxp, gyp, 0.0f, 0.0f);
                sP1[slot] = make_float4(cx, cy, cz, z);
                sP2[slot] = make_float4(__uint_as_float(r2.x), __uint_as_float(r2.y), __uint_as_float(r2.z), op);
            } else {
                const float hx = (-0.5f * L) * cx, hy = (-L) * cy, hz = (-0.5f * L) * cz;
                const float lop = __builtin_amdgcn_logf(op) + 0.014499569695115089f;
                const float d = gxp - bx0f;
                const float b0 = (-2.0f * hx) * d, a1 = hy * d, a0 = __builtin_fmaf(hx * d, d, lop);
                sP0[slot] = make_float4(hx, 0.99f * __uint_as_float(r2.x), 0.99f * __uint_as_float(r2.y), 0.99f * __uint_as_float(r2.z));
                sL[slot] = lop;
                if constexpr (AUX) sZ[slot] = 0.99f * z;
#pragma unroll
                for (int r = 0; r < 8; ++r) {
                    const float dy = gyp - (by0f + (float)r);
                    sT[r * 65 + slot] = make_float2(__builtin_fmaf(-hy, dy, b0), __builtin_fmaf(dy, __builtin_fmaf(dy, hz, a1), a0));
                }
            }
        }
        fill();
        const uint32_t cnt_next = take(vnext);
        if (cnt_next) fetch(vnext, cnt_next);
        __builtin_amdgcn_fence(__ATOMIC_RELEASE, "wavefront");
        __builtin_amdgcn_fence(__ATOMIC_ACQUIRE, "wavefront");
        const uint32_t nrel = (uint32_t)__popcll(m);
        evaluated += nrel;
        const uint32_t trow = (lane >> 3) * 65u;
        const float xlf = (float)(lane & 7u);
        auto walk = [&](auto checked_tag) {
            constexpr bool CHECKED = decltype(checked_tag)::value;
            auto one = [&](uint32_t e, const float4 p0, const float2 tt, const float zz) {
                if (EXACT) {
                    const float dx = p0.x - pxf;
                    const float4 p1 = sP1[e];
                    const float dy = p0.y - pyf;
                    const float4 p2v = sP2[e];
                    const float t1 = p1.x * dx * dx, t2 = p1.z * dy * dy, t3 = p1.y * dx * dy;
                    const float power = -0.5f * (t1 + t2) - t3;
                    const float alpha = wg_min(0.99f, p2v.w * gs_exp(power));
                    const float test = T * (1.0f - alpha);
                    const float cond = (power <= 0.0f && alpha >= c255 && test >= 0.0001f) ? 1.0f : 0.0f;
                    cr += cond * p2v.x * alpha * T;
                    cg += cond * p2v.y * alpha * T;
                    cb += cond * p2v.z * alpha * T;
                    if constexpr (AUX) cd += cond * p1.w * alpha * T;
                    T = cond * test + (1.0f - cond) * T;
                } else {
                    const float pw = __builtin_fmaf(xlf, __builtin_fmaf(xlf, p0.x, tt.x), tt.y);
                    float ea;
                    asm("v_exp_f32_e64 %0, %1 clamp" : "=v"(ea) : "v"(pw));
                    const float k1 = (float)(1.0 / 255.0 / 0.99);
#ifdef GS_PROFILING
                    if (dbg & 32u) {
                        const unsigned long long km = __ballot(ea >= k1);
                        const unsigned long long q0 = 0x000000000F0F0F0Full;
                        fp_lanes += (uint32_t)__popcll(km);
                        fp_quads += (uint32_t)((km & q0) != 0) + (uint32_t)((km & (q0 << 4)) != 0) + (uint32_t)((km & (q0 << 32)) != 0) + (uint32_t)((km & (q0 << 36)) != 0);
                        fp_none += (uint32_t)(km == 0);
                        const unsigned long long lv = __ballot(__builtin_fmaf(-T, c255, T) >= 0.0001f);
                        const unsigned long long kp = __ballot(ea >= k1 && __builtin_fmaf(T * ea, -0.99f, T) >= 0.0001f);
                        fp_live += (uint32_t)__popcll(lv);
                        fp_kept += (uint32_t)__popcll(kp);
                        fp_dead += (uint32_t)((km & lv) == 0);
                        fp_q1 += (uint32_t)(__popcll(lv) <= 16);
                        fp_nokeep += (uint32_t)(kp == 0ull);
                    }
#endif
                    if (CHECKED) {
                        const float wgt = T * ea;
                        const float test = __builtin_fmaf(wgt, -0.99f, T);
                        bool keep = (ea >= k1) && (test >= 0.0001f);
                        keep = keep && (pw <= sL[e]);
                        const float wk = keep ? wgt : 0.0f;
                        cr = __builtin_fmaf(p0.y, wk, cr);
                        cg = __builtin_fmaf(p0.z, wk, cg);
                        cb = __builtin_fmaf(p0.w, wk, cb);
                        if constexpr (AUX) cd = __builtin_fmaf(zz, wk, cd);
                        T = keep ? test : T;
                    } else {
                        float wgt, test;
                        unsigned long long save;
                        if constexpr (AUX)
                            asm(
                                "v_mul_f32_e32 %[wgt], %[T], %[ea]\n\t"
                                "v_fma_f32 %[test], %[wgt], %[m99], %[T]\n\t"
                                "s_mov_b64 %[save], exec\n\t"
                                "v_cmpx_le_f32_e32 vcc, %[k1], %[ea]\n\t"
                                "v_cmpx_le_f32_e32 vcc, %[thr], %[test]\n\t"
                                "v_mov_b32_e32 %[T], %[test]\n\t"
                                "v_fmac_f32_e32 %[cr], %[c0], %[wgt]\n\t"
                                "v_fmac_f32_e32 %[cg], %[c1], %[wgt]\n\t"
                                "v_fmac_f32_e32 %[cb], %[c2], %[wgt]\n\t"
                                "v_fmac_f32_e32 %[cd], %[z], %[wgt]\n\t"
                                "s_mov_b64 exec, %[save]"
                                : [save] "=&s"(save), [wgt] "=&v"(wgt), [test] "=&v"(test), [T] "+v"(T), [cr] "+v"(cr), [cg] "+v"(cg), [cb] "+v"(cb),
                                  [cd] "+v"(cd)
                                : [k1] "s"(k1), [thr] "s"(0.0001f), [m99] "s"(-0.99f), [ea] "v"(ea), [c0] "v"(p0.y), [c1] "v"(p0.z), [c2] "v"(p0.w),
                                  [z] "v"(zz)
                                : "vcc");
                        else
                        asm(
                            "v_mul_f32_e32 %[wgt], %[T], %[ea]\n\t"
                            "v_fma_f32 %[test], %[wgt], %[m99], %[T]\n\t"
                            "s_mov_b64 %[save], exec\n\t"
                            "v_cmpx_le_f32_e32 vcc, %[k1], %[ea]\n\t"
                            "v_cmpx_le_f32_e32 vcc, %[thr], %[test]\n\t"
                            "v_mov_b32_e32 %[T], %[test]\n\t"
                            "v_fmac_f32_e32 %[cr], %[c0], %[wgt]\n\t"
                            "v_fmac_f32_e32 %[cg], %[c1], %[wgt]\n\t"
                            "v_fmac_f32_e32 %[cb], %[c2], %[wgt]\n\t"
                            "s_mov_b64 exec, %[save]"
                            : [save] "=&s"(save), [wgt] "=&v"(wgt), [test] "=&v"(test), [T] "+v"(T), [cr] "+v"(cr), [cg] "+v"(cg), [cb] "+v"(cb)
                            : [k1] "s"(k1), [thr] "s"(0.0001f), [m99] "s"(-0.99f), [ea] "v"(ea), [c0] "v"(p0.y), [c1] "v"(p0.z), [c2] "v"(p0.w)
                            : "vcc");
                    }
                }
            };
            auto group = [&](uint32_t e, auto n_tag) {
                constexpr int G = decltype(n_tag)::value;
                float4 p[G];
                float2 t[G];
                float zz[G];
#pragma unroll
                for (int k = 0; k < G; ++k) {
                    p[k] = sP0[e + k];
                    t[k] = EXACT ? make_float2(0.0f, 0.0f) : sT[trow + e + k];
                    zz[k] = 0.0f;
                    if constexpr (AUX && !EXACT) zz[k] = sZ[e + k];
                }
                __builtin_amdgcn_sched_barrier(0);
#pragma unroll
                for (int k = 0; k < G; ++k) one(e + k, p[k], t[k], zz[k]);
                __builtin_amdgcn_sched_barrier(0);
            };
            uint32_t e = 0;
            if (!EXACT)
                for (; e + 8u <= nrel; e += 8u) group(e, std::integral_constant<int, 8>{});
            for (; e + 4u <= nrel; e += 4u) group(e, std::integral_constant<int, 4>{});
            for (; e < nrel; ++e) group(e, std::integral_constant<int, 1>{});
        };
        if (EXACT || __ballot(npd) != 0ull) walk(std::true_type{});
        else walk(std::false_type{});
        if (EXACT) done = outside || (T * (1.0f - c255) < 0.0001f);
        else done = outside || (__builtin_fmaf(-T, c255, T) < 0.0001f);
        __builtin_amdgcn_fence(__ATOMIC_RELEASE, "wavefront");
        __builtin_amdgcn_fence(__ATOMIC_ACQUIRE, "wavefront");
        if (__ballot(!done) == 0ull) break;
        cnt = cnt_next;
    }
    if (lane == 0 && staged) atomicMax(&tile_depth[lin], staged);
    if (lane == 0 && evaluated) atomicAdd(&ctl->num_evaluated[(b + 1u) & 63u], (unsigned long long)evaluated);
#ifdef GS_PROFILING
    if ((dbg & 32u) && lane == 0) {
        unsigned long long* fp = gs_blend_foot[b & 255u];
        atomicAdd(&fp[0], (unsigned long long)evaluated); atomicAdd(&fp[1], (unsigned long long)fp_lanes);
        atomicAdd(&fp[2], (unsigned long long)fp_quads); atomicAdd(&fp[3], (unsigned long long)fp_none);
        atomicAdd(&fp[4], (unsigned long long)fp_live); atomicAdd(&fp[5], (unsigned long long)fp_kept);
        atomicAdd(&fp[6], (unsigned long long)fp_dead); atomicAdd(&fp[7], (unsigned long long)fp_q1);
        atomicAdd(&fp[8], (unsigned long long)fp_tailn); atomicAdd(&fp[9], (unsigned long long)fp_tailbits); atomicAdd(&fp[10], (unsigned long long)fp_nokeep);
    }
    if (prof && lane == 0) {
        prof[b * 4u + 0u] = t_start;
        prof[b * 4u + 1u] = (uint32_t)__builtin_amdgcn_s_memrealtime();
        prof[b * 4u + 2u] = evaluated;
        prof[b * 4u + 3u] = staged;
    }
#endif
    if (!outside) {
        const float c[3] = {cr, cg, cb};
        uint32_t px = 0xFF000000u;
#pragma unroll
        for (int ch = 0; ch < 3; ++ch) {
            float v = c[ch];
            v = (v != v) ? 0.0f : wg_min(wg_max(v, 0.0f), 1.0f);
            px |= (uint32_t)__builtin_floorf(v * 255.0f + 0.5f) << (8 * ch);
        }
        const uint64_t o = (uint64_t)gy * f.slab_w + (gx - f.px0);
        rgba8[o] = px;
        if (rgbf) {
            rgbf[o * 3 + 0] = cr;
            rgbf[o * 3 + 1] = cg;
            rgbf[o * 3 + 2] = cb;
        }
        if constexpr (AUX) {
            const GsAuxPlanes ap = gs_aux_planes(aux...);
            ap.alpha[o] = 1.0f - T;
            ap.depth[o] = cd;
        }
    }
}

__global__ __launch_bounds__(256) void gs_assemble_kernel(const uint32_t* __restrict__ slabs, uint32_t* __restrict__ image,
                                                           uint32_t width, uint32_t height, const uint32_t* __restrict__ px_bounds,
                                                           uint32_t n_slabs, uint64_t slab_stride_px) {
    const uint64_t t = (uint64_t)blockIdx.x * 256 + threadIdx.x;
    if (t >= (uint64_t)width * height) return;
    const uint32_t y = (uint32_t)(t / width), x = (uint32_t)(t % width);
    uint32_t g = 0;
    while (g + 1 < n_slabs && x >= px_bounds[g + 1]) ++g;
    const uint32_t x0 = px_bounds[g], w = px_bounds[g + 1] - x0;
    const uint64_t slab_off = slab_stride_px ? (uint64_t)g * slab_stride_px : (uint64_t)x0 * height;
    image[t] = slabs[slab_off + (uint64_t)y * w + (x - x0)];
}

__global__ __launch_bounds__(256) void gs_debug_view_kernel(const uint32_t* __restrict__ ranges, GsFrame f, uint32_t view,
                                                             uint32_t* __restrict__ rgba8) {
    const uint64_t t = (uint64_t)blockIdx.x * 256 + threadIdx.x;
    if (t >= (uint64_t)f.slab_w * f.height) return;
    const uint32_t y = (uint32_t)(t / f.slab_w), x = f.px0 + (uint32_t)(t % f.slab_w);
    const uint32_t tile = x / f.tile_size + (y / f.tile_size) * f.ntx;
    const uint32_t start = tile > 0 ? ranges[tile - 1] : 0u, end = ranges[tile];
    const float len = (float)(end - start);
    float c[3];
    if (view == 1u) {
        if (x % f.tile_size != f.tile_size - 1u && y % f.tile_size != f.tile_size - 1u) return;
        c[0] = 1.0f; c[1] = 0.0f; c[2] = 0.0f;
    } else if (view == 2u) {
        c[0] = c[1] = c[2] = len / 1000.0f;
    } else if (view == 3u) {
        c[0] = (float)x / (float)f.width; c[1] = (float)y / (float)f.height; c[2] = 0.0f;
    } else {
        c[0] = c[1] = len / 100.0f; c[2] = 0.0f;
    }
    uint32_t px = 0xFF000000u;
#pragma unroll
    for (int ch = 0; ch < 3; ++ch) {
        const float v = wg_min(wg_max(c[ch], 0.0f), 1.0f);
        px |= (uint32_t)__builtin_floorf(v * 255.0f + 0.5f) << (8 * ch);
    }
    rgba8[t] = px;
}
void gs_launch_debug_view(const uint32_t* ranges, const GsFrame& f, uint32_t view, uint32_t* rgba8, hipStream_t st) {
    const uint64_t total = (uint64_t)f.slab_w * f.height;
    if (!total || !view) return;
    hipLaunchKernelGGL(gs_debug_view_kernel, dim3((uint32_t)((total + 255) / 256)), dim3(256), 0, st, ranges, f, view, rgba8);
}

template <int TS>
static void launch_blend_t(bool exact, bool aux, GsAuxPlanes ap, dim3 grid, hipStream_t st, const uint4* gdata, const uint32_t* values,
                           const uint32_t* ranges, const GsFrame& f, uint32_t* rgba8, float* rgbf, GsControl* ctl, uint32_t dbg, uint32_t id_mask) {
#define GS_WG(E) hipLaunchKernelGGL((gs_blend_kernel<TS, E>), grid, dim3(TS * TS), 0, st, gdata, values, ranges, f, rgba8, rgbf, ctl, dbg, id_mask)
#define GS_WG_AUX(E) hipLaunchKernelGGL((gs_blend_kernel<TS, E, true, GsAuxPlanes>), grid, dim3(TS * TS), 0, st, gdata, values, ranges, f, rgba8, \
                                        rgbf, ctl, dbg, id_mask, ap)
    if (aux) { if (exact) GS_WG_AUX(true); else GS_WG_AUX(false); }
    else { if (exact) GS_WG(true); else GS_WG(false); }
#undef GS_WG
#undef GS_WG_AUX
}
template <int TS>
static void launch_quad_t(bool exact, bool masked, bool aux, GsAuxPlanes ap, uint32_t nblk, uint32_t pad, hipStream_t st, const uint4* g,
                          const uint32_t* values, const uint32_t* ranges, const GsFrame& f, uint32_t* rgba8, float* rgbf, GsControl* ctl,
                          uint32_t* tile_depth, uint32_t dbg, uint32_t* prof) {
#define GS_QUAD(E, M) hipLaunchKernelGGL((gs_blend_quad_kernel<E, TS, M>), dim3(nblk), dim3(64), pad, st, g, values, ranges, f, rgba8, rgbf, ctl, tile_depth, dbg, prof)
#define GS_QUAD_AUX(E, M) hipLaunchKernelGGL((gs_blend_quad_kernel<E, TS, M, true, GsAuxPlanes>), dim3(nblk), dim3(64), pad, st, g, values, ranges, f, \
                                             rgba8, rgbf, ctl, tile_depth, dbg, prof, ap)
    if (aux) {
        if (exact) { if (masked) GS_QUAD_AUX(true, true); else GS_QUAD_AUX(true, false); }
        else { if (masked) GS_QUAD_AUX(false, true); else GS_QUAD_AUX(false, false); }
    } else {
        if (exact) { if (masked) GS_QUAD(true, true); else GS_QUAD(true, false); }
        else { if (masked) GS_QUAD(false, true); else GS_QUAD(false, false); }
    }
#undef GS_QUAD
#undef GS_QUAD_AUX
}
int gs_launch_blend(const void* gdata, const uint32_t* values, const uint32_t* ranges, const GsFrame& f, uint32_t* rgba8, float* rgbf,
                    bool aux, float* alpha, float* depth, GsControl* ctl, uint32_t* tile_depth, bool exact, uint32_t ablation, bool masked,
                    hipStream_t st, uint32_t* prof, uint32_t* prof_blocks) {
    if (aux && (!alpha || !depth)) return -2;
    const GsAuxPlanes ap{alpha, depth};
    uint32_t dbg = ablation;
    const uint32_t id_mask = masked ? GS_ID_MASK : 0xFFFFFFFFu;
    const dim3 grid(f.col1 - f.col0, f.nty);
    if (grid.x == 0 || grid.y == 0) return 1;
    const uint4* g = (const uint4*)gdata;
    switch (f.tile_size) {
    case 8: launch_blend_t<8>(exact, aux, ap, grid, st, g, values, ranges, f, rgba8, rgbf, ctl, dbg, id_mask); return 1;
    case 16:
    case 32: {
        const bool t32 = f.tile_size == 32;
        if (!(dbg & 8u)) {
            const uint32_t slab_tx = grid.x;
            auto widest = [&](uint32_t sw) {
                const uint32_t ns = (slab_tx + sw - 1) / sw, lastw = slab_tx - (ns - 1) * sw;
                uint32_t wmax = 0;
                for (uint32_t x = 0; x < 8 && x < ns; ++x) {
                    const uint32_t n_x = (ns - 1 - x) / 8 + 1, wx = n_x * sw - ((((ns - 1) & 7u) == x) ? sw - lastw : 0u);
                    wmax = wx > wmax ? wx : wmax;
                }
                return wmax;
            };
            uint32_t SW = (dbg >> 8) & 0xffu;
            if (!SW) {
                SW = 1;
                for (uint32_t sw = 3; sw > 1; --sw)
                    if (widest(sw) * 80u <= slab_tx * 11u) { SW = sw; break; }
            }
            dbg = (dbg & 0xffu) | (SW << 8);
            const uint32_t wmax = widest(SW);
            const uint32_t nblk = (t32 ? 128u : 32u) * wmax * grid.y;
#ifdef GS_PROFILING
            const uint32_t pad = (dbg & 64u) ? 20480u - 3072u : (dbg & 128u) ? 10240u - 3072u : 0u;
#else
            const uint32_t pad = 0u;
#endif
            if (prof_blocks) *prof_blocks = nblk;
            if (t32) { launch_quad_t<32>(exact, masked, aux, ap, nblk, pad, st, g, values, ranges, f, rgba8, rgbf, ctl, tile_depth, dbg, prof); return 16; }
            launch_quad_t<16>(exact, masked, aux, ap, nblk, pad, st, g, values, ranges, f, rgba8, rgbf, ctl, tile_depth, dbg, prof);
            return 4;
        }
        if (t32) { launch_blend_t<32>(exact, aux, ap, grid, st, g, values, ranges, f, rgba8, rgbf, ctl, dbg, id_mask); return 1; }
        launch_blend_t<16>(exact, aux, ap, grid, st, g, values, ranges, f, rgba8, rgbf, ctl, dbg, id_mask);
        return 1;
    }
    default: return -1;
    }
}
void gs_launch_assemble(const void* slabs, void* image, uint32_t width, uint32_t height, const uint32_t* d_px_bounds, uint32_t n_slabs,
                        uint64_t slab_stride_px, hipStream_t st) {
    const uint64_t total = (uint64_t)width * height;
    hipLaunchKernelGGL(gs_assemble_kernel, dim3((uint32_t)((total + 255) / 256)), dim3(256), 0, st, (const uint32_t*)slabs, (uint32_t*)image,
                       width, height, d_px_bounds, n_slabs, slab_stride_px);
}
```

### gaussian-splatting-wgpu_amd/csrc/k_rows.hip

```cpp
#include "gs_device.h"
#include "gs_tight.h"

typedef uint32_t gs_item3 __attribute__((ext_vector_type(3), aligned(4)));

#ifndef RA_ITEMS
#define RA_ITEMS 8
#endif
#ifndef RA_WAVES
#define RA_WAVES 8
#endif
#define RA_THREADS (RA_WAVES * 64)
#define RA_TILE (RA_THREADS * RA_ITEMS)
#define RA_AGG (1u << 30)
#define RA_PREFIX (2u << 30)
#define RA_FLAGS (3u << 30)
#define RA_VALUE (~RA_FLAGS)

#ifndef RB_CH
#define RB_CH 512u
#endif
#define RB_IT (RB_CH / 256u)
#ifndef RB_SB
#define RB_SB 2048u
#endif
#define RB_PER (RB_SB / 256u)
#define RB_WSL (RB_SB / 4u)

struct RowSortShared {
    uint32_t hist[RA_WAVES][256];
    uint32_t gbase[256];
    uint32_t tot[256];
    uint32_t dbase[256];
    uint32_t wsum[RA_WAVES];
    uint32_t tile, nvalid;
    union {
        uint32_t it[RA_TILE * 3];
        struct {
            uint32_t goff[RA_TILE + 8], gptr[RA_TILE + 8];
            unsigned short mark[RA_TILE];
        } g;
    } u;
};

__global__ __launch_bounds__(RA_THREADS) void gs_rows_sort_kernel(const uint32_t* __restrict__ arena, const uint4* __restrict__ grec,
                                                                  const uint32_t* __restrict__ chunk_table, uint32_t* __restrict__ rows_out,
                                                                  GsControl* ctl, uint32_t* __restrict__ status, uint32_t row_cap, uint32_t ndig) {
    __shared__ RowSortShared sh;
    const uint32_t hole = ndig < 128u ? 127u : 255u;
    const int nbits = ndig < 128u ? 7 : 8;
    const uint32_t tid = threadIdx.x, lane = tid & 63, w = tid >> 6;
    const unsigned long long lt_mask = (1ull << lane) - 1ull;
    uint32_t n = ctl->num_slots;
    if (n > row_cap) n = row_cap;
    const uint32_t ntiles = (n + RA_TILE - 1) / RA_TILE;
    const uint32_t nvis = ctl->num_visible;
    {
        const uint32_t c = tid < 256u ? gs_rowhist(ctl, tid) : 0u;
        const uint32_t incl = wave_incl_scan(c, lane);
        if (lane == 63) sh.wsum[w] = incl;
        __syncthreads();
        uint32_t b = 0;
        for (uint32_t k = 0; k < w; ++k) b += sh.wsum[k];
        if (tid < 256u) sh.dbase[tid] = b + incl - c;
        __syncthreads();
    }
    for (;;) {
        if (tid == 0) sh.tile = atomicAdd(&ctl->rows_ticket, 1u);
        __syncthreads();
        const uint32_t tile = sh.tile;
        if (tile >= ntiles) break;
        const uint32_t s0 = tile * RA_TILE, s_end = (s0 + RA_TILE < n) ? s0 + RA_TILE : n;
        const uint32_t g0 = chunk_table[s0 >> 10];
        const uint32_t g1 = (s_end < n) ? chunk_table[s_end >> 10] : nvis - 1u;
        uint32_t K = (g1 >= g0) ? g1 - g0 + 1u : 1u;
        if (K > RA_TILE + 8u) K = RA_TILE + 8u;
        for (uint32_t k = tid; k < RA_TILE / 2u; k += RA_THREADS) reinterpret_cast<uint32_t*>(sh.u.g.mark)[k] = 0u;
        __syncthreads();
        for (uint32_t k = tid; k < K; k += RA_THREADS) {
            const uint4 rec = (g0 + k < nvis) ? grec[g0 + k] : make_uint4(0u, 0u, 0xFFFFFFFFu, 0u);
            sh.u.g.goff[k] = rec.z;
            sh.u.g.gptr[k] = rec.w;
            if (rec.z >= s0 && rec.z < s_end) sh.u.g.mark[rec.z - s0] = (unsigned short)(k + 1u);
        }
        __syncthreads();
        uint32_t carry;
        {
            constexpr uint32_t RA_STR = (RA_TILE + 8u + 63u) / 64u;
            static_assert(RA_STR * 64u >= RA_TILE + 8u && RA_STR <= 128u, "the two-level owner search covers the tile's gaussians");
            const uint32_t x0 = s0 + w * (64 * RA_ITEMS);
            const uint32_t m1 = lane * RA_STR;
            const uint32_t c1 = (uint32_t)__popcll(__ballot(m1 < K && sh.u.g.goff[m1 < K ? m1 : 0u] <= x0));
            const uint32_t b1 = (c1 ? c1 - 1u : 0u) * RA_STR;
            uint32_t c2 = 0;
#pragma unroll
            for (uint32_t t2 = 0; t2 < (RA_STR + 63u) / 64u; ++t2) {
                const uint32_t o2 = t2 * 64u + lane, m2 = b1 + o2;
                c2 += (uint32_t)__popcll(__ballot(o2 < RA_STR && m2 < K && sh.u.g.goff[m2 < K ? m2 : 0u] <= x0));
            }
            const uint32_t e = b1 + (c2 ? c2 - 1u : 0u);
            carry = e + 1u;
        }
        uint32_t ix[RA_ITEMS], iy[RA_ITEMS], iz[RA_ITEMS];
        uint32_t rank2[RA_ITEMS / 2];
#pragma unroll
        for (int j = 0; j < RA_ITEMS; ++j) {
            const uint32_t sp = w * (64 * RA_ITEMS) + j * 64 + lane, slot = s0 + sp;
            uint32_t m = wave_incl_max((uint32_t)sh.u.g.mark[sp]);
            m = m > carry ? m : carry;
            carry = (uint32_t)__builtin_amdgcn_readlane((int)m, 63);
            ix[j] = GS_ROW_HOLE; iy[j] = 0u; iz[j] = 0u;
            if (slot < n) {
                const uint32_t k = m - 1u;
                const uint32_t src = sh.u.g.gptr[k] + (slot - sh.u.g.goff[k]);
                if (src < row_cap) {
                    const gs_item3 v = *reinterpret_cast<const gs_item3*>(arena + (uint64_t)src * 3u);
                    ix[j] = v.x; iy[j] = v.y; iz[j] = v.z;
                }
            }
        }
        for (uint32_t k = lane; k < 256; k += 64) sh.hist[w][k] = 0;
        if (tid < 256u) sh.tot[tid] = 0u;
        __syncthreads();
#pragma unroll
        for (int j = 0; j < RA_ITEMS; ++j) atomicAdd(&sh.tot[ix[j] == GS_ROW_HOLE ? hole : (iy[j] & 0xFFu)], 1u);
        __syncthreads();
        if (tid < ndig) st_agent(status + (uint64_t)tile * 256 + tid, (tile == 0 ? RA_PREFIX : RA_AGG) | sh.tot[tid]);
#pragma unroll
        for (int j = 0; j < RA_ITEMS; ++j) {
            const uint32_t d = ix[j] == GS_ROW_HOLE ? hole : (iy[j] & 0xFFu);
            uint32_t plo = 0xFFFFFFFFu, phi = 0xFFFFFFFFu;
#pragma unroll
            for (int b = 0; b < 8; ++b) {
                if (b < nbits) {
                    const uint32_t bit = (d >> b) & 1u;
                    const unsigned long long bal = __ballot(bit != 0u);
                    const uint32_t inv = bit - 1u;
                    plo &= (uint32_t)bal ^ inv;
                    phi &= (uint32_t)(bal >> 32) ^ inv;
                }
            }
            const uint32_t below = __popc(plo & (uint32_t)lt_mask) + __popc(phi & (uint32_t)(lt_mask >> 32));
            const uint32_t cnt = __popc(plo) + __popc(phi);
            const uint32_t pre = sh.hist[w][d];
            __builtin_amdgcn_fence(__ATOMIC_RELEASE, "wavefront");
            if (below == 0) sh.hist[w][d] = pre + cnt;
            __builtin_amdgcn_fence(__ATOMIC_ACQUIRE, "wavefront");
            const uint32_t r = pre + below;
            if (j & 1) rank2[j >> 1] |= r << 16;
            else rank2[j >> 1] = r;
        }
        __syncthreads();
        uint32_t cw[RA_WAVES], total = 0, excl = 0, incl = 0;
        if (tid < 256u) {
#pragma unroll
            for (int k = 0; k < RA_WAVES; ++k) { cw[k] = sh.hist[k][tid]; total += cw[k]; }
            incl = wave_incl_scan(total, lane);
            if (lane == 63) sh.wsum[w] = incl;
            if (tile > 0 && tid < ndig) {
                constexpr int LB = 8;
                bool found = false;
                for (int t = (int)tile - 1; t >= 0 && !found; t -= LB) {
                    uint32_t sv[LB];
#pragma unroll
                    for (int k = 0; k < LB; ++k) sv[k] = (t - k >= 0) ? ld_agent(status + (uint64_t)(t - k) * 256 + tid) : RA_PREFIX;
#pragma unroll
                    for (int k = 0; k < LB; ++k) {
                        if (found) break;
                        uint32_t v = sv[k], spins = 0;
                        while ((v & RA_FLAGS) == 0 && ++spins < GS_SPIN_LIMIT) {
                            __builtin_amdgcn_s_sleep(1);
                            v = ld_agent(status + (uint64_t)(t - k) * 256 + tid);
                        }
                        if ((v & RA_FLAGS) == 0) { ctl->fault = 1u; found = true; break; }
                        excl += v & RA_VALUE;
                        if ((v & RA_FLAGS) == RA_PREFIX) found = true;
                    }
                }
                st_agent(status + (uint64_t)tile * 256 + tid, RA_PREFIX | ((excl + total) & RA_VALUE));
            }
        }
        __syncthreads();
        if (tid < 256u) {
            uint32_t wv = 0;
            for (uint32_t k = 0; k < w; ++k) wv += sh.wsum[k];
            uint32_t run = wv + incl - total;
            if (tid == hole) sh.nvalid = run;
            sh.gbase[tid] = sh.dbase[tid] + excl - run;
#pragma unroll
            for (int k = 0; k < RA_WAVES; ++k) { sh.hist[k][tid] = run; run += cw[k]; }
        }
        __syncthreads();
#pragma unroll
        for (int j = 0; j < RA_ITEMS; ++j) {
            const uint32_t d = ix[j] == GS_ROW_HOLE ? hole : (iy[j] & 0xFFu);
            const uint32_t r = (j & 1) ? (rank2[j >> 1] >> 16) : (rank2[j >> 1] & 0xFFFFu);
            const uint32_t pos = sh.hist[w][d] + r;
            sh.u.it[pos * 3 + 0] = ix[j];
            sh.u.it[pos * 3 + 1] = iy[j];
            sh.u.it[pos * 3 + 2] = iz[j];
        }
        __syncthreads();
        const uint32_t nvalid = sh.nvalid;
#pragma unroll
        for (int j = 0; j < RA_ITEMS; ++j) {
            const uint32_t pos = j * RA_THREADS + tid;
            if (pos < nvalid) {
                gs_item3 v;
                v.x = sh.u.it[pos * 3 + 0]; v.y = sh.u.it[pos * 3 + 1]; v.z = sh.u.it[pos * 3 + 2];
                const uint32_t g = sh.gbase[v.y & 0xFFu] + pos;
                if (g < row_cap) *reinterpret_cast<gs_item3*>(rows_out + (uint64_t)g * 3u) = v;
            }
        }
        __syncthreads();
    }
}

struct RowTables {
    uint32_t ibase[257];
    uint32_t cbase[257];
    uint32_t w4[8];
};
__device__ __forceinline__ void row_tables(RowTables& T, const GsControl* ctl, uint32_t row_cap, uint32_t tid) {
    const uint32_t lane = tid & 63, w = tid >> 6;
    const bool on = tid < 256u;
    const uint32_t c = on ? gs_rowhist(ctl, tid) : 0u;
    const unsigned long long ic = wave_incl_scan64(c, lane);
    if (on && lane == 63) { T.w4[w] = (uint32_t)(ic > 0xFFFFFFFFull ? 0xFFFFFFFFull : ic); }
    __syncthreads();
    uint32_t i0 = 0, cc = 0;
    if (on) {
        unsigned long long b = ic - c;
        for (uint32_t k = 0; k < w; ++k) b += T.w4[k];
        const unsigned long long e = b + c;
        i0 = b > row_cap ? row_cap : (uint32_t)b;
        const uint32_t i1 = e > row_cap ? row_cap : (uint32_t)e;
        cc = i1 - i0;
        T.ibase[tid] = i0;
        if (tid == 255u) T.ibase[256] = i1;
    }
    const uint32_t ch = (cc + RB_CH - 1u) / RB_CH;
    const uint32_t ih = wave_incl_scan(ch, lane);
    if (on && lane == 63) T.w4[4 + w] = ih;
    __syncthreads();
    if (on) {
        uint32_t bh = 0;
        for (uint32_t k = 0; k < w; ++k) bh += T.w4[4 + k];
        T.cbase[tid] = bh + ih - ch;
        if (tid == 255u) T.cbase[256] = bh + ih;
    }
    __syncthreads();
}
__device__ __forceinline__ uint32_t row_of_chunk(const RowTables& T, uint32_t c) {
    const uint32_t lane = threadIdx.x & 63u;
    uint32_t v[4];
#pragma unroll
    for (int k = 0; k < 4; ++k) v[k] = T.cbase[lane + 64u * k];
    uint32_t r = 0;
#pragma unroll
    for (int k = 0; k < 4; ++k) r += (uint32_t)__popcll(__ballot(v[k] <= c && (lane + 64u * k) != 0u));
    return r;
}

__global__ __launch_bounds__(256) void gs_rows_count_kernel(const uint32_t* __restrict__ rows, const GsControl* ctl, uint32_t* __restrict__ M3,
                                                            uint32_t chunk_cap, uint32_t row_cap) {
    __shared__ RowTables T;
    __shared__ int s_diff[257];
    __shared__ uint32_t s_w[4];
    const uint32_t tid = threadIdx.x, lane = tid & 63, w = tid >> 6;
    row_tables(T, ctl, row_cap, tid);
    uint32_t nch = T.cbase[256];
    if (nch > chunk_cap) nch = chunk_cap;
    for (uint32_t c = blockIdx.x; c < nch; c += gridDim.x) {
        const uint32_t r = row_of_chunk(T, c);
        const uint32_t i0 = T.ibase[r] + (c - T.cbase[r]) * RB_CH;
        const uint32_t i1 = (i0 + RB_CH < T.ibase[r + 1]) ? i0 + RB_CH : T.ibase[r + 1];
        s_diff[tid] = 0;
        if (tid == 0) s_diff[256] = 0;
        __syncthreads();
#pragma unroll
        for (int k = 0; k < (int)(RB_CH / 256u); ++k) {
            const uint32_t i = i0 + k * 256u + tid;
            if (i < i1) {
                const uint32_t w1 = rows[(uint64_t)i * 3u + 1u];
                const uint32_t tlo = (w1 >> 8) & 0xFFu, len = ((w1 >> 16) & 0xFFu) + 1u;
                atomicAdd(&s_diff[tlo], 1);
                atomicAdd(&s_diff[tlo + len > 256u ? 256u : tlo + len], -1);
            }
        }
        __syncthreads();
        const uint32_t v = (uint32_t)s_diff[tid];
        const uint32_t incl = wave_incl_scan(v, lane);
        if (lane == 63) s_w[w] = incl;
        __syncthreads();
        uint32_t b = 0;
        for (uint32_t k = 0; k < w; ++k) b += s_w[k];
        M3[(uint64_t)c * 256u + tid] = b + incl;
        __syncthreads();
    }
}

__global__ __launch_bounds__(1024) void gs_rows_scan_kernel(const GsControl* ctl, uint32_t* __restrict__ M3, uint32_t* __restrict__ tileoff,
                                                            uint32_t* __restrict__ rowtot, uint32_t chunk_cap, uint32_t row_cap) {
    __shared__ RowTables T;
    __shared__ unsigned long long s_part[4][256];
    __shared__ unsigned long long s_ex[256];
    __shared__ unsigned long long s_w[4];
    const uint32_t tid = threadIdx.x, c = tid & 255u, p = tid >> 8, r = blockIdx.x;
    row_tables(T, ctl, row_cap, tid);
    uint32_t c0 = T.cbase[r], c1 = T.cbase[r + 1];
    if (c0 > chunk_cap) c0 = chunk_cap;
    if (c1 > chunk_cap) c1 = chunk_cap;
    const uint32_t nch = c1 - c0, per = (nch + 3u) / 4u;
    const uint32_t j0 = c0 + (p * per < nch ? p * per : nch), j1 = c0 + ((p + 1u) * per < nch ? (p + 1u) * per : nch);
    unsigned long long sum = 0;
    for (uint32_t j = j0; j < j1; j += 8u) {
        uint32_t v[8];
#pragma unroll
        for (int k = 0; k < 8; ++k) v[k] = (j + k < j1) ? M3[(uint64_t)(j + k) * 256u + c] : 0u;
#pragma unroll
        for (int k = 0; k < 8; ++k) sum += v[k];
    }
    s_part[p][c] = sum;
    __syncthreads();
    unsigned long long run = 0, tot = 0;
#pragma unroll
    for (int k = 0; k < 4; ++k) { const unsigned long long t = s_part[k][c]; if (k < (int)p) run += t; tot += t; }
    for (uint32_t j = j0; j < j1; j += 8u) {
        uint32_t v[8];
#pragma unroll
        for (int k = 0; k < 8; ++k) v[k] = (j + k < j1) ? M3[(uint64_t)(j + k) * 256u + c] : 0u;
#pragma unroll
        for (int k = 0; k < 8; ++k) {
            if (j + k < j1) M3[(uint64_t)(j + k) * 256u + c] = run > 0xFFFFFFFFull ? 0xFFFFFFFFu : (uint32_t)run;
            run += v[k];
        }
    }
    if (p == 0) {
        const uint32_t lane = tid & 63, w = tid >> 6;
        unsigned long long incl = tot;
#pragma unroll
        for (int d = 1; d < 64; d <<= 1) {
            const uint32_t lo = __shfl_up((uint32_t)incl, d, 64), hi = __shfl_up((uint32_t)(incl >> 32), d, 64);
            if ((int)lane >= d) incl += ((unsigned long long)hi << 32) | lo;
        }
        if (lane == 63) s_w[w] = incl;
        s_ex[c] = incl - tot;
    }
    __syncthreads();
    if (p == 0) {
        const uint32_t w = tid >> 6;
        unsigned long long b = 0, all = 0;
#pragma unroll
        for (int k = 0; k < 4; ++k) { if (k < (int)w) b += s_w[k]; all += s_w[k]; }
        const unsigned long long ex = b + s_ex[c];
        tileoff[r * 256u + c] = ex > 0xFFFFFFFFull ? 0xFFFFFFFFu : (uint32_t)ex;
        if (c == 0) rowtot[r] = all > 0xFFFFFFFFull ? 0xFFFFFFFFu : (uint32_t)all;
    }
}

struct ExpandShared {
    RowTables T;
    uint32_t rbase[257];
    uint32_t w0[RB_CH], w1[RB_CH], w2[RB_CH];
    uint32_t hist[4][256];
    uint32_t gbase[256];
    uint32_t wsum[8];
    uint32_t nvalid, total;
    unsigned char cols[RB_SB];
    union {
        struct { uint32_t P[RB_CH + 1]; unsigned short mark[RB_SB]; } e;
        uint32_t vals[RB_SB];
    } x;
};

__global__ __launch_bounds__(256) void gs_rows_expand_kernel(const uint32_t* __restrict__ rows, GsControl* ctl, const uint32_t* __restrict__ M3,
                                                             const uint32_t* __restrict__ tileoff, const uint32_t* __restrict__ rowtot, GsFrame f,
                                                             uint32_t* __restrict__ values, uint32_t* __restrict__ ranges, uint32_t chunk_cap,
                                                             uint32_t row_cap, uint32_t* sticky, GsReport* rep) {
    __shared__ ExpandShared S;
    const uint32_t tid = threadIdx.x, lane = tid & 63, w = tid >> 6;
    const unsigned long long lt_mask = (1ull << lane) - 1ull;
    const uint32_t ns = f.tile_size >= 16u ? 2u : 1u;
    const uint32_t hole = f.ntx < 128u ? 127u : 255u;
    const int nbits = f.ntx < 128u ? 7 : 8;
    row_tables(S.T, ctl, row_cap, tid);
    {
        const uint32_t v = tid < f.nty ? rowtot[tid] : 0u;
        unsigned long long incl = v;
#pragma unroll
        for (int d = 1; d < 64; d <<= 1) {
            const uint32_t lo = __shfl_up((uint32_t)incl, d, 64), hi = __shfl_up((uint32_t)(incl >> 32), d, 64);
            if ((int)lane >= d) incl += ((unsigned long long)hi << 32) | lo;
        }
        __shared__ unsigned long long s_r[4];
        if (lane == 63) s_r[w] = incl;
        __syncthreads();
        unsigned long long b = 0;
        for (uint32_t k = 0; k < w; ++k) b += s_r[k];
        const unsigned long long ex = b + incl - v;
        S.rbase[tid] = ex > 0xFFFFFFFFull ? 0xFFFFFFFFu : (uint32_t)ex;
        if (tid == 255u) S.rbase[256] = (b + incl) > 0xFFFFFFFFull ? 0xFFFFFFFFu : (uint32_t)(b + incl);
        __syncthreads();
    }
    if (blockIdx.x == 0 && tid == 0) {
        const uint32_t I = S.rbase[256];
        ctl->num_intersections = I;
        ctl->num_items = S.T.ibase[256];
        if (I > f.capacity) ctl->overflow = 1u;
        gs_frame_report(ctl, I, S.T.ibase[256], f.capacity, sticky, rep);
    }
    for (uint32_t r = blockIdx.x; r < f.nty; r += gridDim.x) {
        if (tid < f.ntx) {
            const uint32_t endoff = (tid + 1u < 256u) ? tileoff[r * 256u + tid + 1u] : rowtot[r];
            const unsigned long long e = (unsigned long long)S.rbase[r] + endoff;
            ranges[r * f.ntx + tid] = e > 0xFFFFFFFFull ? 0xFFFFFFFFu : (uint32_t)e;
        }
    }
    uint32_t nch = S.T.cbase[256];
    if (nch > chunk_cap) nch = chunk_cap;
    gs_item3 nit[RB_IT];
    uint32_t n_r = 0, n_ni = 0, n_tstart = 0, n_done = 0;
    auto prefetch = [&](uint32_t c) {
        n_r = row_of_chunk(S.T, c);
        const uint32_t i0 = S.T.ibase[n_r] + (c - S.T.cbase[n_r]) * RB_CH;
        const uint32_t i1 = (i0 + RB_CH < S.T.ibase[n_r + 1]) ? i0 + RB_CH : S.T.ibase[n_r + 1];
        n_ni = i1 - i0;
#pragma unroll
        for (int k = 0; k < (int)RB_IT; ++k) {
            const uint32_t e = tid * RB_IT + k;
            nit[k] = *reinterpret_cast<const gs_item3*>(rows + (uint64_t)(i0 + (e < n_ni ? e : 0u)) * 3u);
        }
        n_tstart = S.rbase[n_r] + tileoff[n_r * 256u + tid];
        n_done = M3[(uint64_t)c * 256u + tid];
    };
    if (blockIdx.x < nch) prefetch(blockIdx.x);
    for (uint32_t c = blockIdx.x; c < nch; c += gridDim.x) {
        const uint32_t ni = n_ni;
        uint32_t len[RB_IT], lsum = 0;
#pragma unroll
        for (int k = 0; k < (int)RB_IT; ++k) {
            const uint32_t e = tid * RB_IT + k;
            len[k] = 0u;
            if (e < ni) {
                S.w0[e] = nit[k].x; S.w1[e] = nit[k].y; S.w2[e] = nit[k].z;
                len[k] = ((nit[k].y >> 16) & 0xFFu) + 1u;
            }
            lsum += len[k];
        }
        const uint32_t tstart = n_tstart;
        uint32_t done = n_done;
        if (c + gridDim.x < nch) prefetch(c + gridDim.x);
        {
            const uint32_t incl = wave_incl_scan(lsum, lane);
            if (lane == 63) S.wsum[w] = incl;
            __syncthreads();
            uint32_t b = 0, all = 0;
#pragma unroll
            for (int k = 0; k < 4; ++k) { if (k < (int)w) b += S.wsum[k]; all += S.wsum[k]; }
            uint32_t run = b + incl - lsum;
#pragma unroll
            for (int k = 0; k < (int)RB_IT; ++k) { S.x.e.P[tid * RB_IT + k] = run; run += len[k]; }
            if (tid == 0) { S.x.e.P[RB_CH] = all; S.total = all; }
        }
        __syncthreads();
        const uint32_t ninst = S.total;
        for (uint32_t s0 = 0; s0 < ninst; s0 += RB_SB) {
            if (s0) {
                __syncthreads();
                uint32_t l2[RB_IT], ls = 0;
#pragma unroll
                for (int k = 0; k < (int)RB_IT; ++k) { const uint32_t e = tid * RB_IT + k; l2[k] = e < ni ? ((S.w1[e] >> 16) & 0xFFu) + 1u : 0u; ls += l2[k]; }
                const uint32_t incl = wave_incl_scan(ls, lane);
                if (lane == 63) S.wsum[w] = incl;
                __syncthreads();
                uint32_t b = 0;
#pragma unroll
                for (int k = 0; k < 4; ++k) if (k < (int)w) b += S.wsum[k];
                uint32_t run = b + incl - ls;
#pragma unroll
                for (int k = 0; k < (int)RB_IT; ++k) { S.x.e.P[tid * RB_IT + k] = run; run += l2[k]; }
                if (tid == 0) S.x.e.P[RB_CH] = ninst;
            }
            for (uint32_t k = tid; k < RB_SB / 2u; k += 256u) reinterpret_cast<uint32_t*>(S.x.e.mark)[k] = 0u;
            for (uint32_t k = lane; k < 256; k += 64) S.hist[w][k] = 0u;
            __syncthreads();
#pragma unroll
            for (int k = 0; k < (int)RB_IT; ++k) {
                const uint32_t e = tid * RB_IT + k;
                if (e < ni) {
                    const uint32_t p0 = S.x.e.P[e];
                    if (p0 >= s0 && p0 < s0 + RB_SB) S.x.e.mark[p0 - s0] = (unsigned short)(e + 1u);
                }
            }
            __syncthreads();
            uint32_t carry;
            {
                const uint32_t x0 = s0 + w * RB_WSL;
                uint32_t pv[RB_CH / 64u];
#pragma unroll
                for (int k = 0; k < (int)(RB_CH / 64u); ++k) pv[k] = S.x.e.P[lane + 64u * k];
                uint32_t e = 0;
#pragma unroll
                for (int k = 0; k < (int)(RB_CH / 64u); ++k) {
                    const uint32_t m = lane + 64u * k;
                    e += (uint32_t)__popcll(__ballot(m != 0u && m < ni && pv[k] <= x0));
                }
                carry = e + 1u;
            }
            uint32_t val[RB_PER], col4[RB_PER / 4u];
            uint32_t rank2[RB_PER / 2u];
#pragma unroll
            for (int j = 0; j < (int)(RB_PER / 4u); ++j) col4[j] = 0u;
            const uint32_t wfirst = s0 + w * RB_WSL;
            const uint32_t jn = wfirst >= ninst ? 0u : ((ninst - wfirst + 63u) / 64u < RB_PER ? (ninst - wfirst + 63u) / 64u : RB_PER);
#pragma unroll
            for (int j = 0; j < (int)RB_PER; ++j) {
                if ((uint32_t)j >= jn) break;
                const uint32_t sp = w * RB_WSL + j * 64u + lane, x = s0 + sp;
                uint32_t m = wave_incl_max((uint32_t)S.x.e.mark[sp]);
                m = m > carry ? m : carry;
                carry = (uint32_t)__builtin_amdgcn_readlane((int)m, 63);
                uint32_t d = hole;
                val[j] = 0u;
                if (x < ninst) {
                    const uint32_t e = m - 1u;
                    const uint32_t q = x - S.x.e.P[e], i1w = S.w1[e];
                    d = ((i1w >> 8) & 0xFFu) + q;
                    val[j] = (S.w0[e] & GS_ID_MASK) | (tight_item_mask(S.w2[e], q, ns) << GS_ID_BITS);
                }
                col4[j >> 2] |= d << (8 * (j & 3));
            }
#pragma unroll
            for (int j = 0; j < (int)RB_PER; ++j) {
                if ((uint32_t)j >= jn) break;
                const uint32_t d = (col4[j >> 2] >> (8 * (j & 3))) & 0xFFu;
                uint32_t plo = 0xFFFFFFFFu, phi = 0xFFFFFFFFu;
#pragma unroll
                for (int b = 0; b < 8; ++b) {
                    if (b < nbits) {
                        const uint32_t bit = (d >> b) & 1u;
                        const unsigned long long bal = __ballot(bit != 0u);
                        const uint32_t inv = bit - 1u;
                        plo &= (uint32_t)bal ^ inv;
                        phi &= (uint32_t)(bal >> 32) ^ inv;
                    }
                }
                const uint32_t below = __popc(plo & (uint32_t)lt_mask) + __popc(phi & (uint32_t)(lt_mask >> 32));
                const uint32_t cnt = __popc(plo) + __popc(phi);
                const uint32_t pre = S.hist[w][d];
                __builtin_amdgcn_fence(__ATOMIC_RELEASE, "wavefront");
                if (below == 0) S.hist[w][d] = pre + cnt;
                __builtin_amdgcn_fence(__ATOMIC_ACQUIRE, "wavefront");
                const uint32_t rr = pre + below;
                if (j & 1) rank2[j >> 1] |= rr << 16;
                else rank2[j >> 1] = rr;
            }
            __syncthreads();
            {
                uint32_t cw[4], total = 0;
#pragma unroll
                for (int k = 0; k < 4; ++k) { cw[k] = S.hist[k][tid]; total += cw[k]; }
                const uint32_t incl = wave_incl_scan(total, lane);
                if (lane == 63) S.wsum[4 + w] = incl;
                __syncthreads();
                uint32_t b = 0;
#pragma unroll
                for (int k = 0; k < 4; ++k) if (k < (int)w) b += S.wsum[4 + k];
                uint32_t run = b + incl - total;
                if (tid == hole) S.nvalid = run;
                S.gbase[tid] = tstart + done - run;
                done += total;
#pragma unroll
                for (int k = 0; k < 4; ++k) { S.hist[k][tid] = run; run += cw[k]; }
            }
            __syncthreads();
#pragma unroll
            for (int j = 0; j < (int)RB_PER; ++j) {
                if ((uint32_t)j >= jn) break;
                const uint32_t d = (col4[j >> 2] >> (8 * (j & 3))) & 0xFFu;
                const uint32_t rr = (j & 1) ? (rank2[j >> 1] >> 16) : (rank2[j >> 1] & 0xFFFFu);
                const uint32_t pos = S.hist[w][d] + rr;
                S.x.vals[pos] = val[j];
                S.cols[pos] = (unsigned char)d;
            }
            __syncthreads();
            const uint32_t nvalid = S.nvalid;
#pragma unroll
            for (int j = 0; j < (int)RB_PER; ++j) {
                const uint32_t pos = j * 256u + tid;
                if (pos < nvalid) {
                    const uint32_t dst = S.gbase[S.cols[pos]] + pos;
                    if (dst < f.capacity) values[dst] = S.x.vals[pos];
                }
            }
        }
        __syncthreads();
    }
}

__global__ __launch_bounds__(256) void gs_rows_rebuild_keys_kernel(const uint32_t* __restrict__ ranges, uint32_t T, const uint32_t* __restrict__ vals,
                                                                   const uint32_t* __restrict__ counts, uint32_t count, uint32_t n,
                                                                   uint32_t* __restrict__ keys) {
    for (uint32_t i = blockIdx.x * 256u + threadIdx.x; i < count; i += gridDim.x * 256u) {
        uint32_t lo = 0, hi = T;
        while (lo < hi) {
            const uint32_t mid = (lo + hi) >> 1;
            if (ranges[mid] > i) hi = mid; else lo = mid + 1u;
        }
        const uint32_t g = vals[i] & GS_ID_MASK;
        keys[i] = lo * 1000u + (g < n ? counts[g] >> GS_COUNT_BITS : 0u);
    }
}

#ifndef RB_CNT_WG
#define RB_CNT_WG 8u
#endif
#ifndef RB_EXP_WG
#define RB_EXP_WG 6u
#endif
uint32_t gs_rows_sort_tiles(uint64_t row_cap) { return (uint32_t)((row_cap + RA_TILE - 1) / RA_TILE); }
uint32_t gs_rows_chunks(uint64_t row_cap) { return (uint32_t)(row_cap / RB_CH + 256u); }
void gs_launch_rows(const uint32_t* arena, const void* grec, const uint32_t* chunk_table, uint32_t* rows_sorted, GsControl* ctl, uint32_t* sort_status, uint32_t row_cap,
                    uint32_t* M3, uint32_t* tileoff, uint32_t* rowtot, const GsFrame& f, uint32_t* values, uint32_t* ranges, uint32_t cus,
                    uint32_t* sticky, GsReport* rep, hipStream_t st, void (*mark)(void*, int), void* mark_arg) {
    const uint32_t chunk_cap = gs_rows_chunks(row_cap);
    if (!cus) cus = 1;
    hipLaunchKernelGGL(gs_rows_sort_kernel, dim3(cus * 3u), dim3(RA_THREADS), 0, st, arena, (const uint4*)grec, chunk_table, rows_sorted, ctl, sort_status,
                       row_cap, f.nty);
    if (mark) mark(mark_arg, 3);
    hipLaunchKernelGGL(gs_rows_count_kernel, dim3(cus * RB_CNT_WG), dim3(256), 0, st, (const uint32_t*)rows_sorted, (const GsControl*)ctl, M3, chunk_cap, row_cap);
    hipLaunchKernelGGL(gs_rows_scan_kernel, dim3(f.nty), dim3(1024), 0, st, (const GsControl*)ctl, M3, tileoff, rowtot, chunk_cap, row_cap);
    hipLaunchKernelGGL(gs_rows_expand_kernel, dim3(cus * RB_EXP_WG), dim3(256), 0, st, (const uint32_t*)rows_sorted, ctl, (const uint32_t*)M3,
                       (const uint32_t*)tileoff, (const uint32_t*)rowtot, f, values, ranges, chunk_cap, row_cap, sticky, rep);
}
void gs_launch_rows_rebuild_keys(const uint32_t* ranges, uint32_t T, const uint32_t* vals, const uint32_t* counts, uint32_t count, uint32_t n,
                                 uint32_t* keys, hipStream_t st) {
    if (!count) return;
    const uint32_t blocks = (count + 255u) / 256u;
    hipLaunchKernelGGL(gs_rows_rebuild_keys_kernel, dim3(blocks < 4096u ? blocks : 4096u), dim3(256), 0, st, ranges, T, vals, counts, count, n, keys);
}
```

Before: 1321 frames/s.

## Precompute row tables once, pack expand records, and enable blend pixel test

```diff
diff --git a/gaussian-splatting-wgpu_amd/csrc/gs_context.hip b/gaussian-splatting-wgpu_amd/csrc/gs_context.hip
--- a/gaussian-splatting-wgpu_amd/csrc/gs_context.hip
+++ b/gaussian-splatting-wgpu_amd/csrc/gs_context.hip
@@ -128,6 +128,7 @@
     HIP_TRY(hipMalloc(c->d_pxb.out(), 65 * 4));
     HIP_TRY(hipMalloc(c->tileoff.out(), 256 * 256 * 4));
     HIP_TRY(hipMalloc(c->rowtot.out(), 256 * 4));
+    HIP_TRY(hipMalloc(c->row_tab.out(), (size_t)gs_rows_table_words() * 4));
     HIP_TRY(hipMalloc(c->sticky.out(), 4 * 4));
     HIP_TRY(hipMemset(c->sticky, 0, 4 * 4));
     HIP_TRY(hipHostMalloc(c->h_rep.out(), sizeof(GsReport), hipHostMallocDefault));
diff --git a/gaussian-splatting-wgpu_amd/csrc/gs_frame.hip b/gaussian-splatting-wgpu_amd/csrc/gs_frame.hip
--- a/gaussian-splatting-wgpu_amd/csrc/gs_frame.hip
+++ b/gaussian-splatting-wgpu_amd/csrc/gs_frame.hip
@@ -52,7 +52,7 @@
         gs_launch_gsort(c->counts, c->rowptr, c->n, c->gsort_scratch, c->grec, c->chunk_table, (uint32_t)gs_emit_chunks(std::max(c->capacity, c->row_cap)),
                         &c->ctl->num_visible, &c->ctl->num_slots, c->grid_persist, st);
         mark(c, 2);
-        gs_launch_rows(c->arena, c->grec, c->chunk_table, c->rows_sorted, c->ctl, c->rows_status, (uint32_t)c->row_cap, c->M3, c->tileoff, c->rowtot, f, c->valsA,
+        gs_launch_rows(c->arena, c->grec, c->chunk_table, c->rows_sorted, c->ctl, c->rows_status, (uint32_t)c->row_cap, c->row_tab, c->M3, c->tileoff, c->rowtot, f, c->valsA,
                        c->ranges, c->grid_persist / 4u, c->sticky, c->h_rep, st, mark_cb, c);
         nt.keysS = nullptr;
         nt.valsS = c->valsA;
diff --git a/gaussian-splatting-wgpu_amd/csrc/gs_kernels.h b/gaussian-splatting-wgpu_amd/csrc/gs_kernels.h
--- a/gaussian-splatting-wgpu_amd/csrc/gs_kernels.h
+++ b/gaussian-splatting-wgpu_amd/csrc/gs_kernels.h
@@ -46,8 +46,9 @@
                      uint32_t* tot_visible, uint32_t* tot_quantity, uint32_t grid, hipStream_t st);
 uint32_t gs_rows_sort_tiles(uint64_t row_cap);
 uint32_t gs_rows_chunks(uint64_t row_cap);
+uint32_t gs_rows_table_words(void);
 void gs_launch_rows(const uint32_t* arena, const void* grec, const uint32_t* chunk_table, uint32_t* rows_sorted, GsControl* ctl, uint32_t* sort_status, uint32_t row_cap,
-                    uint32_t* M3, uint32_t* tileoff, uint32_t* rowtot, const GsFrame& f, uint32_t* values, uint32_t* ranges, uint32_t cus,
+                    uint32_t* row_tab, uint32_t* M3, uint32_t* tileoff, uint32_t* rowtot, const GsFrame& f, uint32_t* values, uint32_t* ranges, uint32_t cus,
                     uint32_t* sticky, GsReport* rep, hipStream_t st, void (*mark)(void*, int), void* mark_arg);
 void gs_launch_rows_rebuild_keys(const uint32_t* ranges, uint32_t T, const uint32_t* vals, const uint32_t* counts, uint32_t count, uint32_t n,
                                  uint32_t* keys, hipStream_t st);
diff --git a/gaussian-splatting-wgpu_amd/csrc/gs_runtime.h b/gaussian-splatting-wgpu_amd/csrc/gs_runtime.h
--- a/gaussian-splatting-wgpu_amd/csrc/gs_runtime.h
+++ b/gaussian-splatting-wgpu_amd/csrc/gs_runtime.h
@@ -110,6 +110,7 @@
     uint64_t row_cap = 0;
     DevBuf<uint32_t> arena, rows_sorted, M3;
     DevBuf<uint32_t> tileoff, rowtot;
+    DevBuf<uint32_t> row_tab;
     DevBuf<> ctl_mem;
     size_t ctl_bytes = 0;
     size_t ctl_bytes_tight = 0;
diff --git a/gaussian-splatting-wgpu_amd/csrc/gs_tight.h b/gaussian-splatting-wgpu_amd/csrc/gs_tight.h
--- a/gaussian-splatting-wgpu_amd/csrc/gs_tight.h
+++ b/gaussian-splatting-wgpu_amd/csrc/gs_tight.h
@@ -217,3 +217,24 @@
     }
     return (uint32_t)(l0 <= q && (q < h0 || h0 == 255u));
 }
+
+#define GS_FIELD_COLS 32u
+__device__ __forceinline__ uint32_t tight_strip_field(uint32_t l, uint32_t h) {
+    if (l >= GS_FIELD_COLS) return 0u;
+    return (0xFFFFFFFFu << l) & (h >= GS_FIELD_COLS ? 0xFFFFFFFFu : (1u << h) - 1u);
+}
+struct TightFields { uint32_t U, L, wide; };
+__device__ __forceinline__ TightFields tight_item_fields(uint32_t w2, uint32_t len, uint32_t ns) {
+    TightFields f;
+    f.wide = len * ns > GS_FIELD_COLS ? 1u : 0u;
+    f.U = tight_strip_field(w2 & 0xFFu, (w2 >> 8) & 0xFFu);
+    f.L = ns == 2u ? tight_strip_field((w2 >> 16) & 0xFFu, w2 >> 24) : 0u;
+    return f;
+}
+__device__ __forceinline__ uint32_t tight_field_mask(uint32_t U, uint32_t L, uint32_t q, uint32_t ns) {
+    const uint32_t sh = (q << (ns - 1u)) & 31u;
+    return ((U >> sh) & (ns == 2u ? 3u : 1u)) | (((L >> sh) & 3u) << 2);
+}
+__device__ __forceinline__ uint32_t tight_item_mask_staged(const TightFields& f, uint32_t w2, uint32_t q, uint32_t ns) {
+    return f.wide ? tight_item_mask(w2, q, ns) : tight_field_mask(f.U, f.L, q, ns);
+}
diff --git a/gaussian-splatting-wgpu_amd/csrc/k_blend.hip b/gaussian-splatting-wgpu_amd/csrc/k_blend.hip
--- a/gaussian-splatting-wgpu_amd/csrc/k_blend.hip
+++ b/gaussian-splatting-wgpu_amd/csrc/k_blend.hip
@@ -254,6 +254,9 @@
     constexpr uint32_t BPR = TS / 8, NB = BPR * BPR;
 #ifdef GS_PROFILING
     const uint32_t t_start = prof ? (uint32_t)__builtin_amdgcn_s_memrealtime() : 0u;
+#endif
+#ifndef GS_BLEND_PIXTEST
+#define GS_BLEND_PIXTEST 8
 #endif
 #ifndef GS_L_OFF_T
 #define GS_L_OFF_T 0
@@ -410,7 +413,7 @@
                     if (Tmax * (1.0f - alo) < 0.0000999f) rel = false;
                 }
 #endif
-#ifdef GS_BLEND_PIXTEST
+#if GS_BLEND_PIXTEST
                 if (rel && pd && !nocull && (uint32_t)__popcll(lv) <= GS_BLEND_PIXTEST) {
                     bool any = false;
                     for (unsigned long long mm = lv; mm; mm &= mm - 1ull) {
diff --git a/gaussian-splatting-wgpu_amd/csrc/k_rows.hip b/gaussian-splatting-wgpu_amd/csrc/k_rows.hip
--- a/gaussian-splatting-wgpu_amd/csrc/k_rows.hip
+++ b/gaussian-splatting-wgpu_amd/csrc/k_rows.hip
@@ -26,200 +26,13 @@
 #define RB_PER (RB_SB / 256u)
 #define RB_WSL (RB_SB / 4u)
 
-struct RowSortShared {
-    uint32_t hist[RA_WAVES][256];
-    uint32_t gbase[256];
-    uint32_t tot[256];
-    uint32_t dbase[256];
-    uint32_t wsum[RA_WAVES];
-    uint32_t tile, nvalid;
-    union {
-        uint32_t it[RA_TILE * 3];
-        struct {
-            uint32_t goff[RA_TILE + 8], gptr[RA_TILE + 8];
-            unsigned short mark[RA_TILE];
-        } g;
-    } u;
-};
-
-__global__ __launch_bounds__(RA_THREADS) void gs_rows_sort_kernel(const uint32_t* __restrict__ arena, const uint4* __restrict__ grec,
-                                                                  const uint32_t* __restrict__ chunk_table, uint32_t* __restrict__ rows_out,
-                                                                  GsControl* ctl, uint32_t* __restrict__ status, uint32_t row_cap, uint32_t ndig) {
-    __shared__ RowSortShared sh;
-    const uint32_t hole = ndig < 128u ? 127u : 255u;
-    const int nbits = ndig < 128u ? 7 : 8;
-    const uint32_t tid = threadIdx.x, lane = tid & 63, w = tid >> 6;
-    const unsigned long long lt_mask = (1ull << lane) - 1ull;
-    uint32_t n = ctl->num_slots;
-    if (n > row_cap) n = row_cap;
-    const uint32_t ntiles = (n + RA_TILE - 1) / RA_TILE;
-    const uint32_t nvis = ctl->num_visible;
-    {
-        const uint32_t c = tid < 256u ? gs_rowhist(ctl, tid) : 0u;
-        const uint32_t incl = wave_incl_scan(c, lane);
-        if (lane == 63) sh.wsum[w] = incl;
-        __syncthreads();
-        uint32_t b = 0;
-        for (uint32_t k = 0; k < w; ++k) b += sh.wsum[k];
-        if (tid < 256u) sh.dbase[tid] = b + incl - c;
-        __syncthreads();
-    }
-    for (;;) {
-        if (tid == 0) sh.tile = atomicAdd(&ctl->rows_ticket, 1u);
-        __syncthreads();
-        const uint32_t tile = sh.tile;
-        if (tile >= ntiles) break;
-        const uint32_t s0 = tile * RA_TILE, s_end = (s0 + RA_TILE < n) ? s0 + RA_TILE : n;
-        const uint32_t g0 = chunk_table[s0 >> 10];
-        const uint32_t g1 = (s_end < n) ? chunk_table[s_end >> 10] : nvis - 1u;
-        uint32_t K = (g1 >= g0) ? g1 - g0 + 1u : 1u;
-        if (K > RA_TILE + 8u) K = RA_TILE + 8u;
-        for (uint32_t k = tid; k < RA_TILE / 2u; k += RA_THREADS) reinterpret_cast<uint32_t*>(sh.u.g.mark)[k] = 0u;
-        __syncthreads();
-        for (uint32_t k = tid; k < K; k += RA_THREADS) {
-            const uint4 rec = (g0 + k < nvis) ? grec[g0 + k] : make_uint4(0u, 0u, 0xFFFFFFFFu, 0u);
-            sh.u.g.goff[k] = rec.z;
-            sh.u.g.gptr[k] = rec.w;
-            if (rec.z >= s0 && rec.z < s_end) sh.u.g.mark[rec.z - s0] = (unsigned short)(k + 1u);
-        }
-        __syncthreads();
-        uint32_t carry;
-        {
-            constexpr uint32_t RA_STR = (RA_TILE + 8u + 63u) / 64u;
-            static_assert(RA_STR * 64u >= RA_TILE + 8u && RA_STR <= 128u, "the two-level owner search covers the tile's gaussians");
-            const uint32_t x0 = s0 + w * (64 * RA_ITEMS);
-            const uint32_t m1 = lane * RA_STR;
-            const uint32_t c1 = (uint32_t)__popcll(__ballot(m1 < K && sh.u.g.goff[m1 < K ? m1 : 0u] <= x0));
-            const uint32_t b1 = (c1 ? c1 - 1u : 0u) * RA_STR;
-            uint32_t c2 = 0;
-#pragma unroll
-            for (uint32_t t2 = 0; t2 < (RA_STR + 63u) / 64u; ++t2) {
-                const uint32_t o2 = t2 * 64u + lane, m2 = b1 + o2;
-                c2 += (uint32_t)__popcll(__ballot(o2 < RA_STR && m2 < K && sh.u.g.goff[m2 < K ? m2 : 0u] <= x0));
-            }
-            const uint32_t e = b1 + (c2 ? c2 - 1u : 0u);
-            carry = e + 1u;
-        }
-        uint32_t ix[RA_ITEMS], iy[RA_ITEMS], iz[RA_ITEMS];
-        uint32_t rank2[RA_ITEMS / 2];
-#pragma unroll
-        for (int j = 0; j < RA_ITEMS; ++j) {
-            const uint32_t sp = w * (64 * RA_ITEMS) + j * 64 + lane, slot = s0 + sp;
-            uint32_t m = wave_incl_max((uint32_t)sh.u.g.mark[sp]);
-            m = m > carry ? m : carry;
-            carry = (uint32_t)__builtin_amdgcn_readlane((int)m, 63);
-            ix[j] = GS_ROW_HOLE; iy[j] = 0u; iz[j] = 0u;
-            if (slot < n) {
-                const uint32_t k = m - 1u;
-                const uint32_t src = sh.u.g.gptr[k] + (slot - sh.u.g.goff[k]);
-                if (src < row_cap) {
-                    const gs_item3 v = *reinterpret_cast<const gs_item3*>(arena + (uint64_t)src * 3u);
-                    ix[j] = v.x; iy[j] = v.y; iz[j] = v.z;
-                }
-            }
-        }
-        for (uint32_t k = lane; k < 256; k += 64) sh.hist[w][k] = 0;
-        if (tid < 256u) sh.tot[tid] = 0u;
-        __syncthreads();
-#pragma unroll
-        for (int j = 0; j < RA_ITEMS; ++j) atomicAdd(&sh.tot[ix[j] == GS_ROW_HOLE ? hole : (iy[j] & 0xFFu)], 1u);
-        __syncthreads();
-        if (tid < ndig) st_agent(status + (uint64_t)tile * 256 + tid, (tile == 0 ? RA_PREFIX : RA_AGG) | sh.tot[tid]);
-#pragma unroll
-        for (int j = 0; j < RA_ITEMS; ++j) {
-            const uint32_t d = ix[j] == GS_ROW_HOLE ? hole : (iy[j] & 0xFFu);
-            uint32_t plo = 0xFFFFFFFFu, phi = 0xFFFFFFFFu;
-#pragma unroll
-            for (int b = 0; b < 8; ++b) {
-                if (b < nbits) {
-                    const uint32_t bit = (d >> b) & 1u;
-                    const unsigned long long bal = __ballot(bit != 0u);
-                    const uint32_t inv = bit - 1u;
-                    plo &= (uint32_t)bal ^ inv;
-                    phi &= (uint32_t)(bal >> 32) ^ inv;
-                }
-            }
-            const uint32_t below = __popc(plo & (uint32_t)lt_mask) + __popc(phi & (uint32_t)(lt_mask >> 32));
-            const uint32_t cnt = __popc(plo) + __popc(phi);
-            const uint32_t pre = sh.hist[w][d];
-            __builtin_amdgcn_fence(__ATOMIC_RELEASE, "wavefront");
-            if (below == 0) sh.hist[w][d] = pre + cnt;
-            __builtin_amdgcn_fence(__ATOMIC_ACQUIRE, "wavefront");
-            const uint32_t r = pre + below;
-            if (j & 1) rank2[j >> 1] |= r << 16;
-            else rank2[j >> 1] = r;
-        }
-        __syncthreads();
-        uint32_t cw[RA_WAVES], total = 0, excl = 0, incl = 0;
-        if (tid < 256u) {
-#pragma unroll
-            for (int k = 0; k < RA_WAVES; ++k) { cw[k] = sh.hist[k][tid]; total += cw[k]; }
-            incl = wave_incl_scan(total, lane);
-            if (lane == 63) sh.wsum[w] = incl;
-            if (tile > 0 && tid < ndig) {
-                constexpr int LB = 8;
-                bool found = false;
-                for (int t = (int)tile - 1; t >= 0 && !found; t -= LB) {
-                    uint32_t sv[LB];
-#pragma unroll
-                    for (int k = 0; k < LB; ++k) sv[k] = (t - k >= 0) ? ld_agent(status + (uint64_t)(t - k) * 256 + tid) : RA_PREFIX;
-#pragma unroll
-                    for (int k = 0; k < LB; ++k) {
-                        if (found) break;
-                        uint32_t v = sv[k], spins = 0;
-                        while ((v & RA_FLAGS) == 0 && ++spins < GS_SPIN_LIMIT) {
-                            __builtin_amdgcn_s_sleep(1);
-                            v = ld_agent(status + (uint64_t)(t - k) * 256 + tid);
-                        }
-                        if ((v & RA_FLAGS) == 0) { ctl->fault = 1u; found = true; break; }
-                        excl += v & RA_VALUE;
-                        if ((v & RA_FLAGS) == RA_PREFIX) found = true;
-                    }
-                }
-                st_agent(status + (uint64_t)tile * 256 + tid, RA_PREFIX | ((excl + total) & RA_VALUE));
-            }
-        }
-        __syncthreads();
-        if (tid < 256u) {
-            uint32_t wv = 0;
-            for (uint32_t k = 0; k < w; ++k) wv += sh.wsum[k];
-            uint32_t run = wv + incl - total;
-            if (tid == hole) sh.nvalid = run;
-            sh.gbase[tid] = sh.dbase[tid] + excl - run;
-#pragma unroll
-            for (int k = 0; k < RA_WAVES; ++k) { sh.hist[k][tid] = run; run += cw[k]; }
-        }
-        __syncthreads();
-#pragma unroll
-        for (int j = 0; j < RA_ITEMS; ++j) {
-            const uint32_t d = ix[j] == GS_ROW_HOLE ? hole : (iy[j] & 0xFFu);
-            const uint32_t r = (j & 1) ? (rank2[j >> 1] >> 16) : (rank2[j >> 1] & 0xFFFFu);
-            const uint32_t pos = sh.hist[w][d] + r;
-            sh.u.it[pos * 3 + 0] = ix[j];
-            sh.u.it[pos * 3 + 1] = iy[j];
-            sh.u.it[pos * 3 + 2] = iz[j];
-        }
-        __syncthreads();
-        const uint32_t nvalid = sh.nvalid;
-#pragma unroll
-        for (int j = 0; j < RA_ITEMS; ++j) {
-            const uint32_t pos = j * RA_THREADS + tid;
-            if (pos < nvalid) {
-                gs_item3 v;
-                v.x = sh.u.it[pos * 3 + 0]; v.y = sh.u.it[pos * 3 + 1]; v.z = sh.u.it[pos * 3 + 2];
-                const uint32_t g = sh.gbase[v.y & 0xFFu] + pos;
-                if (g < row_cap) *reinterpret_cast<gs_item3*>(rows_out + (uint64_t)g * 3u) = v;
-            }
-        }
-        __syncthreads();
-    }
-}
-
 struct RowTables {
     uint32_t ibase[257];
     uint32_t cbase[257];
     uint32_t w4[8];
 };
+#define RB_TAB_WORDS 514u
+static_assert(offsetof(RowTables, cbase) == 257u * 4u && offsetof(RowTables, w4) == RB_TAB_WORDS * 4u, "ibase and cbase are the stored words, in this order");
 __device__ __forceinline__ void row_tables(RowTables& T, const GsControl* ctl, uint32_t row_cap, uint32_t tid) {
     const uint32_t lane = tid & 63, w = tid >> 6;
     const bool on = tid < 256u;
@@ -250,6 +63,206 @@
     }
     __syncthreads();
 }
+__device__ __forceinline__ void row_tables_load(RowTables& T, const uint32_t* __restrict__ tab, uint32_t tid, uint32_t nthreads) {
+    for (uint32_t k = tid; k < RB_TAB_WORDS; k += nthreads) T.ibase[k] = tab[k];
+}
+
+struct RowSortShared {
+    uint32_t hist[RA_WAVES][256];
+    uint32_t gbase[256];
+    uint32_t tot[256];
+    uint32_t dbase[256];
+    uint32_t wsum[RA_WAVES];
+    uint32_t tile, nvalid;
+    union {
+        uint32_t it[RA_TILE * 3];
+        struct {
+            uint32_t goff[RA_TILE + 8], gptr[RA_TILE + 8];
+            unsigned short mark[RA_TILE];
+        } g;
+        RowTables rt;
+    } u;
+};
+
+__global__ __launch_bounds__(RA_THREADS) void gs_rows_sort_kernel(const uint32_t* __restrict__ arena, const uint4* __restrict__ grec,
+                                                                  const uint32_t* __restrict__ chunk_table, uint32_t* __restrict__ rows_out,
+                                                                  GsControl* ctl, uint32_t* __restrict__ status, uint32_t row_cap, uint32_t ndig,
+                                                                  uint32_t* __restrict__ row_tab) {
+    __shared__ RowSortShared sh;
+    const uint32_t hole = ndig < 128u ? 127u : 255u;
+    const int nbits = ndig < 128u ? 7 : 8;
+    const uint32_t tid = threadIdx.x, lane = tid & 63, w = tid >> 6;
+    const unsigned long long lt_mask = (1ull << lane) - 1ull;
+    uint32_t n = ctl->num_slots;
+    if (n > row_cap) n = row_cap;
+    const uint32_t ntiles = (n + RA_TILE - 1) / RA_TILE;
+    const uint32_t nvis = ctl->num_visible;
+    {
+        const uint32_t c = tid < 256u ? gs_rowhist(ctl, tid) : 0u;
+        const uint32_t incl = wave_incl_scan(c, lane);
+        if (lane == 63) sh.wsum[w] = incl;
+        __syncthreads();
+        uint32_t b = 0;
+        for (uint32_t k = 0; k < w; ++k) b += sh.wsum[k];
+        if (tid < 256u) sh.dbase[tid] = b + incl - c;
+        __syncthreads();
+    }
+    if (blockIdx.x == 0) {
+        row_tables(sh.u.rt, ctl, row_cap, tid);
+        for (uint32_t k = tid; k < RB_TAB_WORDS; k += RA_THREADS) row_tab[k] = sh.u.rt.ibase[k];
+        __syncthreads();
+    }
+    for (;;) {
+        if (tid == 0) sh.tile = atomicAdd(&ctl->rows_ticket, 1u);
+        __syncthreads();
+        const uint32_t tile = sh.tile;
+        if (tile >= ntiles) break;
+        const uint32_t s0 = tile * RA_TILE, s_end = (s0 + RA_TILE < n) ? s0 + RA_TILE : n;
+        const uint32_t g0 = chunk_table[s0 >> 10];
+        const uint32_t g1 = (s_end < n) ? chunk_table[s_end >> 10] : nvis - 1u;
+        uint32_t K = (g1 >= g0) ? g1 - g0 + 1u : 1u;
+        if (K > RA_TILE + 8u) K = RA_TILE + 8u;
+        for (uint32_t k = tid; k < RA_TILE / 2u; k += RA_THREADS) reinterpret_cast<uint32_t*>(sh.u.g.mark)[k] = 0u;
+        __syncthreads();
+        for (uint32_t k = tid; k < K; k += RA_THREADS) {
+            const uint4 rec = (g0 + k < nvis) ? grec[g0 + k] : make_uint4(0u, 0u, 0xFFFFFFFFu, 0u);
+            sh.u.g.goff[k] = rec.z;
+            sh.u.g.gptr[k] = rec.w;
+            if (rec.z >= s0 && rec.z < s_end) sh.u.g.mark[rec.z - s0] = (unsigned short)(k + 1u);
+        }
+        __syncthreads();
+        uint32_t carry;
+        {
+            constexpr uint32_t RA_STR = (RA_TILE + 8u + 63u) / 64u;
+            static_assert(RA_STR * 64u >= RA_TILE + 8u && RA_STR <= 128u, "the two-level owner search covers the tile's gaussians");
+            const uint32_t x0 = s0 + w * (64 * RA_ITEMS);
+            const uint32_t m1 = lane * RA_STR;
+            const uint32_t c1 = (uint32_t)__popcll(__ballot(m1 < K && sh.u.g.goff[m1 < K ? m1 : 0u] <= x0));
+            const uint32_t b1 = (c1 ? c1 - 1u : 0u) * RA_STR;
+            uint32_t c2 = 0;
+#pragma unroll
+            for (uint32_t t2 = 0; t2 < (RA_STR + 63u) / 64u; ++t2) {
+                const uint32_t o2 = t2 * 64u + lane, m2 = b1 + o2;
+                c2 += (uint32_t)__popcll(__ballot(o2 < RA_STR && m2 < K && sh.u.g.goff[m2 < K ? m2 : 0u] <= x0));
+            }
+            const uint32_t e = b1 + (c2 ? c2 - 1u : 0u);
+            carry = e + 1u;
+        }
+        uint32_t ix[RA_ITEMS], iy[RA_ITEMS], iz[RA_ITEMS];
+        uint32_t rank2[RA_ITEMS / 2];
+#pragma unroll
+        for (int j = 0; j < RA_ITEMS; ++j) {
+            const uint32_t sp = w * (64 * RA_ITEMS) + j * 64 + lane, slot = s0 + sp;
+            uint32_t m = wave_incl_max((uint32_t)sh.u.g.mark[sp]);
+            m = m > carry ? m : carry;
+            carry = (uint32_t)__builtin_amdgcn_readlane((int)m, 63);
+            ix[j] = GS_ROW_HOLE; iy[j] = 0u; iz[j] = 0u;
+            if (slot < n) {
+                const uint32_t k = m - 1u;
+                const uint32_t src = sh.u.g.gptr[k] + (slot - sh.u.g.goff[k]);
+                if (src < row_cap) {
+                    const gs_item3 v = *reinterpret_cast<const gs_item3*>(arena + (uint64_t)src * 3u);
+                    ix[j] = v.x; iy[j] = v.y; iz[j] = v.z;
+                }
+            }
+        }
+        for (uint32_t k = lane; k < 256; k += 64) sh.hist[w][k] = 0;
+        if (tid < 256u) sh.tot[tid] = 0u;
+        __syncthreads();
+#pragma unroll
+        for (int j = 0; j < RA_ITEMS; ++j) atomicAdd(&sh.tot[ix[j] == GS_ROW_HOLE ? hole : (iy[j] & 0xFFu)], 1u);
+        __syncthreads();
+        if (tid < ndig) st_agent(status + (uint64_t)tile * 256 + tid, (tile == 0 ? RA_PREFIX : RA_AGG) | sh.tot[tid]);
+#pragma unroll
+        for (int j = 0; j < RA_ITEMS; ++j) {
+            const uint32_t d = ix[j] == GS_ROW_HOLE ? hole : (iy[j] & 0xFFu);
+            uint32_t plo = 0xFFFFFFFFu, phi = 0xFFFFFFFFu;
+#pragma unroll
+            for (int b = 0; b < 8; ++b) {
+                if (b < nbits) {
+                    const uint32_t bit = (d >> b) & 1u;
+                    const unsigned long long bal = __ballot(bit != 0u);
+                    const uint32_t inv = bit - 1u;
+                    plo &= (uint32_t)bal ^ inv;
+                    phi &= (uint32_t)(bal >> 32) ^ inv;
+                }
+            }
+            const uint32_t below = __popc(plo & (uint32_t)lt_mask) + __popc(phi & (uint32_t)(lt_mask >> 32));
+            const uint32_t cnt = __popc(plo) + __popc(phi);
+            const uint32_t pre = sh.hist[w][d];
+            __builtin_amdgcn_fence(__ATOMIC_RELEASE, "wavefront");
+            if (below == 0) sh.hist[w][d] = pre + cnt;
+            __builtin_amdgcn_fence(__ATOMIC_ACQUIRE, "wavefront");
+            const uint32_t r = pre + below;
+            if (j & 1) rank2[j >> 1] |= r << 16;
+            else rank2[j >> 1] = r;
+        }
+        __syncthreads();
+        uint32_t cw[RA_WAVES], total = 0, excl = 0, incl = 0;
+        if (tid < 256u) {
+#pragma unroll
+            for (int k = 0; k < RA_WAVES; ++k) { cw[k] = sh.hist[k][tid]; total += cw[k]; }
+            incl = wave_incl_scan(total, lane);
+            if (lane == 63) sh.wsum[w] = incl;
+            if (tile > 0 && tid < ndig) {
+                constexpr int LB = 8;
+                bool found = false;
+                for (int t = (int)tile - 1; t >= 0 && !found; t -= LB) {
+                    uint32_t sv[LB];
+#pragma unroll
+                    for (int k = 0; k < LB; ++k) sv[k] = (t - k >= 0) ? ld_agent(status + (uint64_t)(t - k) * 256 + tid) : RA_PREFIX;
+#pragma unroll
+                    for (int k = 0; k < LB; ++k) {
+                        if (found) break;
+                        uint32_t v = sv[k], spins = 0;
+                        while ((v & RA_FLAGS) == 0 && ++spins < GS_SPIN_LIMIT) {
+                            __builtin_amdgcn_s_sleep(1);
+                            v = ld_agent(status + (uint64_t)(t - k) * 256 + tid);
+                        }
+                        if ((v & RA_FLAGS) == 0) { ctl->fault = 1u; found = true; break; }
+                        excl += v & RA_VALUE;
+                        if ((v & RA_FLAGS) == RA_PREFIX) found = true;
+                    }
+                }
+                st_agent(status + (uint64_t)tile * 256 + tid, RA_PREFIX | ((excl + total) & RA_VALUE));
+            }
+        }
+        __syncthreads();
+        if (tid < 256u) {
+            uint32_t wv = 0;
+            for (uint32_t k = 0; k < w; ++k) wv += sh.wsum[k];
+            uint32_t run = wv + incl - total;
+            if (tid == hole) sh.nvalid = run;
+            sh.gbase[tid] = sh.dbase[tid] + excl - run;
+#pragma unroll
+            for (int k = 0; k < RA_WAVES; ++k) { sh.hist[k][tid] = run; run += cw[k]; }
+        }
+        __syncthreads();
+#pragma unroll
+        for (int j = 0; j < RA_ITEMS; ++j) {
+            const uint32_t d = ix[j] == GS_ROW_HOLE ? hole : (iy[j] & 0xFFu);
+            const uint32_t r = (j & 1) ? (rank2[j >> 1] >> 16) : (rank2[j >> 1] & 0xFFFFu);
+            const uint32_t pos = sh.hist[w][d] + r;
+            sh.u.it[pos * 3 + 0] = ix[j];
+            sh.u.it[pos * 3 + 1] = iy[j];
+            sh.u.it[pos * 3 + 2] = iz[j];
+        }
+        __syncthreads();
+        const uint32_t nvalid = sh.nvalid;
+#pragma unroll
+        for (int j = 0; j < RA_ITEMS; ++j) {
+            const uint32_t pos = j * RA_THREADS + tid;
+            if (pos < nvalid) {
+                gs_item3 v;
+                v.x = sh.u.it[pos * 3 + 0]; v.y = sh.u.it[pos * 3 + 1]; v.z = sh.u.it[pos * 3 + 2];
+                const uint32_t g = sh.gbase[v.y & 0xFFu] + pos;
+                if (g < row_cap) *reinterpret_cast<gs_item3*>(rows_out + (uint64_t)g * 3u) = v;
+            }
+        }
+        __syncthreads();
+    }
+}
+
 __device__ __forceinline__ uint32_t row_of_chunk(const RowTables& T, uint32_t c) {
     const uint32_t lane = threadIdx.x & 63u;
     uint32_t v[4];
@@ -261,13 +274,14 @@
     return r;
 }
 
-__global__ __launch_bounds__(256) void gs_rows_count_kernel(const uint32_t* __restrict__ rows, const GsControl* ctl, uint32_t* __restrict__ M3,
-                                                            uint32_t chunk_cap, uint32_t row_cap) {
+__global__ __launch_bounds__(256) void gs_rows_count_kernel(const uint32_t* __restrict__ rows, const uint32_t* __restrict__ row_tab, uint32_t* __restrict__ M3,
+                                                            uint32_t chunk_cap) {
     __shared__ RowTables T;
     __shared__ int s_diff[257];
     __shared__ uint32_t s_w[4];
     const uint32_t tid = threadIdx.x, lane = tid & 63, w = tid >> 6;
-    row_tables(T, ctl, row_cap, tid);
+    row_tables_load(T, row_tab, tid, 256u);
+    __syncthreads();
     uint32_t nch = T.cbase[256];
     if (nch > chunk_cap) nch = chunk_cap;
     for (uint32_t c = blockIdx.x; c < nch; c += gridDim.x) {
@@ -299,14 +313,15 @@
     }
 }
 
-__global__ __launch_bounds__(1024) void gs_rows_scan_kernel(const GsControl* ctl, uint32_t* __restrict__ M3, uint32_t* __restrict__ tileoff,
-                                                            uint32_t* __restrict__ rowtot, uint32_t chunk_cap, uint32_t row_cap) {
+__global__ __launch_bounds__(1024) void gs_rows_scan_kernel(const uint32_t* __restrict__ row_tab, uint32_t* __restrict__ M3, uint32_t* __restrict__ tileoff,
+                                                            uint32_t* __restrict__ rowtot, uint32_t chunk_cap) {
     __shared__ RowTables T;
     __shared__ unsigned long long s_part[4][256];
     __shared__ unsigned long long s_ex[256];
     __shared__ unsigned long long s_w[4];
     const uint32_t tid = threadIdx.x, c = tid & 255u, p = tid >> 8, r = blockIdx.x;
-    row_tables(T, ctl, row_cap, tid);
+    row_tables_load(T, row_tab, tid, 1024u);
+    __syncthreads();
     uint32_t c0 = T.cbase[r], c1 = T.cbase[r + 1];
     if (c0 > chunk_cap) c0 = chunk_cap;
     if (c1 > chunk_cap) c1 = chunk_cap;
@@ -361,7 +376,7 @@
 struct ExpandShared {
     RowTables T;
     uint32_t rbase[257];
-    uint32_t w0[RB_CH], w1[RB_CH], w2[RB_CH];
+    uint4 rec[RB_CH];
     uint32_t hist[4][256];
     uint32_t gbase[256];
     uint32_t wsum[8];
@@ -372,18 +387,21 @@
         uint32_t vals[RB_SB];
     } x;
 };
+#define RB_REC_PBITS 18
+static_assert(RB_CH * 256u < (1u << RB_REC_PBITS), "an item's prefix inside its chunk fits the record");
+static_assert(sizeof(ExpandShared) + 32u <= (160u * 1024u / 6u) / 1280u * 1280u, "six expansion workgroups fit a CU's LDS");
 
 __global__ __launch_bounds__(256) void gs_rows_expand_kernel(const uint32_t* __restrict__ rows, GsControl* ctl, const uint32_t* __restrict__ M3,
                                                              const uint32_t* __restrict__ tileoff, const uint32_t* __restrict__ rowtot, GsFrame f,
                                                              uint32_t* __restrict__ values, uint32_t* __restrict__ ranges, uint32_t chunk_cap,
-                                                             uint32_t row_cap, uint32_t* sticky, GsReport* rep) {
+                                                             const uint32_t* __restrict__ row_tab, uint32_t* sticky, GsReport* rep) {
     __shared__ ExpandShared S;
     const uint32_t tid = threadIdx.x, lane = tid & 63, w = tid >> 6;
     const unsigned long long lt_mask = (1ull << lane) - 1ull;
     const uint32_t ns = f.tile_size >= 16u ? 2u : 1u;
     const uint32_t hole = f.ntx < 128u ? 127u : 255u;
     const int nbits = f.ntx < 128u ? 7 : 8;
-    row_tables(S.T, ctl, row_cap, tid);
+    row_tables_load(S.T, row_tab, tid, 256u);
     {
         const uint32_t v = tid < f.nty ? rowtot[tid] : 0u;
         unsigned long long incl = v;
@@ -436,14 +454,18 @@
     if (blockIdx.x < nch) prefetch(blockIdx.x);
     for (uint32_t c = blockIdx.x; c < nch; c += gridDim.x) {
         const uint32_t ni = n_ni;
-        uint32_t len[RB_IT], lsum = 0;
+        uint32_t len[RB_IT], cw3[RB_IT], lsum = 0;
 #pragma unroll
         for (int k = 0; k < (int)RB_IT; ++k) {
             const uint32_t e = tid * RB_IT + k;
             len[k] = 0u;
+            cw3[k] = 0u;
             if (e < ni) {
-                S.w0[e] = nit[k].x; S.w1[e] = nit[k].y; S.w2[e] = nit[k].z;
                 len[k] = ((nit[k].y >> 16) & 0xFFu) + 1u;
+                const TightFields tf = tight_item_fields(nit[k].z, len[k], ns);
+                cw3[k] = (((nit[k].y >> 8) & 0xFFu) << RB_REC_PBITS) | (tf.wide << 31);
+                uint32_t* const r = reinterpret_cast<uint32_t*>(&S.rec[e]);
+                r[0] = nit[k].x & GS_ID_MASK; r[1] = tf.wide ? nit[k].z : tf.U; r[2] = tf.L;
             }
             lsum += len[k];
         }
@@ -459,7 +481,12 @@
             for (int k = 0; k < 4; ++k) { if (k < (int)w) b += S.wsum[k]; all += S.wsum[k]; }
             uint32_t run = b + incl - lsum;
 #pragma unroll
-            for (int k = 0; k < (int)RB_IT; ++k) { S.x.e.P[tid * RB_IT + k] = run; run += len[k]; }
+            for (int k = 0; k < (int)RB_IT; ++k) {
+                const uint32_t e = tid * RB_IT + k;
+                S.x.e.P[e] = run;
+                S.rec[e].w = cw3[k] | run;
+                run += len[k];
+            }
             if (tid == 0) { S.x.e.P[RB_CH] = all; S.total = all; }
         }
         __syncthreads();
@@ -467,18 +494,8 @@
         for (uint32_t s0 = 0; s0 < ninst; s0 += RB_SB) {
             if (s0) {
                 __syncthreads();
-                uint32_t l2[RB_IT], ls = 0;
-#pragma unroll
-                for (int k = 0; k < (int)RB_IT; ++k) { const uint32_t e = tid * RB_IT + k; l2[k] = e < ni ? ((S.w1[e] >> 16) & 0xFFu) + 1u : 0u; ls += l2[k]; }
-                const uint32_t incl = wave_incl_scan(ls, lane);
-                if (lane == 63) S.wsum[w] = incl;
-                __syncthreads();
-                uint32_t b = 0;
-#pragma unroll
-                for (int k = 0; k < 4; ++k) if (k < (int)w) b += S.wsum[k];
-                uint32_t run = b + incl - ls;
-#pragma unroll
-                for (int k = 0; k < (int)RB_IT; ++k) { S.x.e.P[tid * RB_IT + k] = run; run += l2[k]; }
+#pragma unroll
+                for (int k = 0; k < (int)RB_IT; ++k) S.x.e.P[tid * RB_IT + k] = S.rec[tid * RB_IT + k].w & ((1u << RB_REC_PBITS) - 1u);
                 if (tid == 0) S.x.e.P[RB_CH] = ninst;
             }
             for (uint32_t k = tid; k < RB_SB / 2u; k += 256u) reinterpret_cast<uint32_t*>(S.x.e.mark)[k] = 0u;
@@ -488,7 +505,7 @@
             for (int k = 0; k < (int)RB_IT; ++k) {
                 const uint32_t e = tid * RB_IT + k;
                 if (e < ni) {
-                    const uint32_t p0 = S.x.e.P[e];
+                    const uint32_t p0 = S.rec[e].w & ((1u << RB_REC_PBITS) - 1u);
                     if (p0 >= s0 && p0 < s0 + RB_SB) S.x.e.mark[p0 - s0] = (unsigned short)(e + 1u);
                 }
             }
@@ -523,10 +540,14 @@
                 uint32_t d = hole;
                 val[j] = 0u;
                 if (x < ninst) {
-                    const uint32_t e = m - 1u;
-                    const uint32_t q = x - S.x.e.P[e], i1w = S.w1[e];
-                    d = ((i1w >> 8) & 0xFFu) + q;
-                    val[j] = (S.w0[e] & GS_ID_MASK) | (tight_item_mask(S.w2[e], q, ns) << GS_ID_BITS);
+                    const uint4 it = S.rec[m - 1u];
+                    const uint32_t q = x - (it.w & ((1u << RB_REC_PBITS) - 1u));
+                    d = ((it.w >> RB_REC_PBITS) & 0xFFu) + q;
+                    uint32_t mk = tight_field_mask(it.y, it.z, q, ns);
+                    if (__builtin_amdgcn_ballot_w64((int)it.w < 0) != 0ull) {
+                        if ((int)it.w < 0) mk = tight_item_mask(it.y, q, ns);
+                    }
+                    val[j] = it.x | (mk << GS_ID_BITS);
                 }
                 col4[j >> 2] |= d << (8 * (j & 3));
             }
@@ -620,18 +641,19 @@
 #endif
 uint32_t gs_rows_sort_tiles(uint64_t row_cap) { return (uint32_t)((row_cap + RA_TILE - 1) / RA_TILE); }
 uint32_t gs_rows_chunks(uint64_t row_cap) { return (uint32_t)(row_cap / RB_CH + 256u); }
+uint32_t gs_rows_table_words(void) { return RB_TAB_WORDS; }
 void gs_launch_rows(const uint32_t* arena, const void* grec, const uint32_t* chunk_table, uint32_t* rows_sorted, GsControl* ctl, uint32_t* sort_status, uint32_t row_cap,
-                    uint32_t* M3, uint32_t* tileoff, uint32_t* rowtot, const GsFrame& f, uint32_t* values, uint32_t* ranges, uint32_t cus,
+                    uint32_t* row_tab, uint32_t* M3, uint32_t* tileoff, uint32_t* rowtot, const GsFrame& f, uint32_t* values, uint32_t* ranges, uint32_t cus,
                     uint32_t* sticky, GsReport* rep, hipStream_t st, void (*mark)(void*, int), void* mark_arg) {
     const uint32_t chunk_cap = gs_rows_chunks(row_cap);
     if (!cus) cus = 1;
     hipLaunchKernelGGL(gs_rows_sort_kernel, dim3(cus * 3u), dim3(RA_THREADS), 0, st, arena, (const uint4*)grec, chunk_table, rows_sorted, ctl, sort_status,
-                       row_cap, f.nty);
+                       row_cap, f.nty, row_tab);
     if (mark) mark(mark_arg, 3);
-    hipLaunchKernelGGL(gs_rows_count_kernel, dim3(cus * RB_CNT_WG), dim3(256), 0, st, (const uint32_t*)rows_sorted, (const GsControl*)ctl, M3, chunk_cap, row_cap);
-    hipLaunchKernelGGL(gs_rows_scan_kernel, dim3(f.nty), dim3(1024), 0, st, (const GsControl*)ctl, M3, tileoff, rowtot, chunk_cap, row_cap);
+    hipLaunchKernelGGL(gs_rows_count_kernel, dim3(cus * RB_CNT_WG), dim3(256), 0, st, (const uint32_t*)rows_sorted, (const uint32_t*)row_tab, M3, chunk_cap);
+    hipLaunchKernelGGL(gs_rows_scan_kernel, dim3(f.nty), dim3(1024), 0, st, (const uint32_t*)row_tab, M3, tileoff, rowtot, chunk_cap);
     hipLaunchKernelGGL(gs_rows_expand_kernel, dim3(cus * RB_EXP_WG), dim3(256), 0, st, (const uint32_t*)rows_sorted, ctl, (const uint32_t*)M3,
-                       (const uint32_t*)tileoff, (const uint32_t*)rowtot, f, values, ranges, chunk_cap, row_cap, sticky, rep);
+                       (const uint32_t*)tileoff, (const uint32_t*)rowtot, f, values, ranges, chunk_cap, (const uint32_t*)row_tab, sticky, rep);
 }
 void gs_launch_rows_rebuild_keys(const uint32_t* ranges, uint32_t T, const uint32_t* vals, const uint32_t* counts, uint32_t count, uint32_t n,
                                  uint32_t* keys, hipStream_t st) {
```

Result: no change. 1330 frames/s, median of 6 (+0.7%).
